# MinhZou/SNGNN

Measured on AMD Instinct MI355X. Metric: similarity-aggregation edges/sec, higher is better.
Workload: dtype f32; 1 GPU; ogbn-arxiv-sized synthetic graph, SNGNN_Plus aggregation forward, top_k=16, thr=0.0, self-loops removed; nodes_per_gpu=169343, edges_per_gpu=1163820, channels=40, parallelism=single GPU

## Files before the change

### include/sngnn_hip.h

```cpp
#ifndef SNGNN_HIP_H
#define SNGNN_HIP_H

#include <stdint.h>

#ifdef __cplusplus
extern "C" {
#endif

#define SNGNN_OK            0
#define SNGNN_EINVAL       -1
#define SNGNN_ERANGE       -2
#define SNGNN_EHIP         -3
#define SNGNN_ENOMEM       -4

#define SNGNN_UNSELECTED   (-4.0f)

#define SNGNN_MAX_CHANNELS  512

const char *sngnn_last_error(void);
const char *sngnn_build_info(void);

typedef struct sngnn_graph sngnn_graph_t;

#define SNGNN_LOOPS_REPLACE 2
int sngnn_graph_create(const int64_t *edge_index_dev, int64_t E, int64_t N,
                       int add_loops, int remove_loops, void *stream,
                       sngnn_graph_t **out_graph);
int sngnn_graph_create_partition(const int64_t *edge_index_dev, int64_t E,
                                 int64_t N_total, int64_t row_begin,
                                 int64_t row_end, int add_loops, int remove_loops,
                                 void *stream, sngnn_graph_t **out_graph);
void sngnn_graph_destroy(sngnn_graph_t *g);

int64_t sngnn_graph_num_nodes(const sngnn_graph_t *g);
int64_t sngnn_graph_num_total_nodes(const sngnn_graph_t *g);
int64_t sngnn_graph_row_offset(const sngnn_graph_t *g);
int64_t sngnn_graph_num_edges(const sngnn_graph_t *g);
int64_t sngnn_graph_max_in_degree(const sngnn_graph_t *g);
int64_t sngnn_graph_src_min(const sngnn_graph_t *g);
int64_t sngnn_graph_num_fused_nodes(const sngnn_graph_t *g);
int64_t sngnn_graph_workspace_bytes(const sngnn_graph_t *g, int C);

int sngnn_graph_copy_array(const sngnn_graph_t *g, int which, void *host_dst);
const void *sngnn_graph_array_dev(const sngnn_graph_t *g, int which);
int64_t sngnn_graph_array_len(const sngnn_graph_t *g, int which);

int sngnn_agg_forward(const sngnn_graph_t *g, const float *h, int C, int top_k,
                      float thr, float *out, float *wsel, float *inv_norm,
                      int32_t *sel_src, float *sel_w, void *workspace,
                      void *stream);

int sngnn_normalize_rows(const float *h, int64_t rows, int C, float *n, float *nrm,
                         void *stream);
int64_t sngnn_filter_row_bytes(int C);
int sngnn_normalize_rows_filter(const float *h, int64_t rows, int C, float *n, float *nrm,
                                void *filt, void *stream);
int sngnn_agg_forward_prepared(const sngnn_graph_t *g, const float *n, const float *nrm,
                               const void *filt, int C, int top_k, float thr, float *out,
                               float *wsel, float *inv_norm, int32_t *sel_src, float *sel_w,
                               void *workspace, void *stream);

typedef struct sngnn_epilogue {
    const float *bias;
    const unsigned char *keep;
    float keep_scale;
    int relu;
    const void *seed;
    float p;
    void *kept_bits;
    const int64_t *head_y;
    const unsigned char *head_sel;
    int head_sets;
    int head_out_mode;
    int64_t head_n_a, head_n_b;
    float *head_metrics;
    void *head_workspace;
    int no_filter;
} sngnn_epilogue_t;
int64_t sngnn_agg_head_workspace_bytes(const sngnn_graph_t *g);
int sngnn_agg_head_supported(const sngnn_graph_t *g, int C, int top_k);
int sngnn_agg_forward_epilogue(const sngnn_graph_t *g, const float *h, int C, int top_k, float thr,
                               const sngnn_epilogue_t *epi, float *out, float *wsel, float *inv_norm,
                               void *workspace, void *stream);
int sngnn_agg_forward_prepared_epilogue(const sngnn_graph_t *g, const float *n, const float *nrm,
                                        const void *filt, int C, int top_k, float thr,
                                        const sngnn_epilogue_t *epi, float *out, float *wsel,
                                        float *inv_norm, void *workspace, void *stream);
int sngnn_filter_enable(int mode);
int sngnn_filter_wanted(const sngnn_graph_t *g, int C, int top_k, float thr);
int sngnn_agg_forward_rows(const sngnn_graph_t *g, const float *n, const float *nrm,
                           const void *filt, int C, int top_k, float thr,
                           const uint8_t *row_flag, int row_want, float *out, float *wsel,
                           float *inv_norm, void *workspace, void *stream);
int sngnn_tuning_set(int which, int value);
int sngnn_last_forward_finalize_workgroups(void);
int sngnn_filter_pair_scores(const void *filt, int C, const int64_t *pair_a, const int64_t *pair_b,
                             int64_t n_pairs, float *out, void *stream);
int sngnn_agg_forward_normalized(const sngnn_graph_t *g, const float *n, const float *nrm,
                                 int C, int top_k, float thr, float *out, float *wsel,
                                 float *inv_norm, int32_t *sel_src, float *sel_w,
                                 void *workspace, void *stream);

int sngnn_agg_backward(const sngnn_graph_t *g, const float *h, int C,
                       const float *grad_out, const float *wsel, float *grad_h,
                       void *workspace, void *stream);
int sngnn_agg_backward_topk(const sngnn_graph_t *g, const float *h, int C,
                            const float *grad_out, const float *wsel, int top_k, float *grad_h,
                            void *workspace, void *stream);
int sngnn_agg_kept_bits_supported(const sngnn_graph_t *g, int C, int top_k);
int64_t sngnn_graph_kept_bits_bytes(const sngnn_graph_t *g);
int sngnn_agg_backward_bits(const sngnn_graph_t *g, const float *h, int C, const float *grad_out,
                            const void *kept_bits, int top_k, float *grad_h, void *workspace, void *stream);

#define SNGNN_DTYPE_F16 1
#define SNGNN_DTYPE_BF16 2
int sngnn_agg_forward_half(const sngnn_graph_t *g, const void *h, int dtype, int C, int top_k, float thr,
                           void *out, float *wsel, float *inv_norm, int32_t *sel_src, float *sel_w,
                           void *workspace, void *stream);
int sngnn_agg_backward_half(const sngnn_graph_t *g, const void *h, int dtype, int C, const void *grad_out,
                            const float *wsel, int top_k, void *grad_h, void *workspace, void *stream);

int sngnn_attn_forward(const sngnn_graph_t *g, const float *h, int C, float *out,
                       float *alpha, void *workspace, void *stream);
int sngnn_attn_backward(const sngnn_graph_t *g, const float *h, int C,
                        const float *grad_out, const float *alpha, float *grad_h,
                        void *workspace, void *stream);

int sngnn_signed_forward(const sngnn_graph_t *g, const float *wh, int C, const float *coef,
                         const float *c2, float *out, float *s, void *workspace, void *stream);
int sngnn_signed_backward(const sngnn_graph_t *g, const float *wh, int C, const float *grad_out,
                          const float *coef, const float *s, const float *c2, float *grad_wh, float *u,
                          void *workspace, void *stream);

int sngnn_attn_forward_half(const sngnn_graph_t *g, const void *h, int dtype, int C, void *out,
                            float *alpha, void *workspace, void *stream);
int sngnn_attn_backward_half(const sngnn_graph_t *g, const void *h, int dtype, int C, const void *grad_out,
                             const float *alpha, void *grad_h, void *workspace, void *stream);
int sngnn_signed_forward_half(const sngnn_graph_t *g, const void *wh, int dtype, int C, const float *coef,
                              const float *c2, void *out, float *s, void *workspace, void *stream);
int sngnn_signed_backward_half(const sngnn_graph_t *g, const void *wh, int dtype, int C, const void *grad_out,
                               const float *coef, const float *s, const float *c2, void *grad_wh, float *u,
                               void *workspace, void *stream);

int64_t sngnn_blend_workspace_bytes(void);
int sngnn_blend_forward(const float *out0, const float *out1, const float *beta, int64_t n,
                        float *out, void *stream);
int sngnn_blend_backward(const float *grad_out, const float *out0, const float *out1,
                         const float *beta, int64_t n, float *grad0, float *grad1,
                         float *grad_beta, void *workspace, void *stream);
int sngnn_blend_forward_epilogue(const float *out0, const float *out1, const float *beta, int64_t n,
                                 const sngnn_epilogue_t *epi, float *out, void *stream);
int sngnn_blend_backward_epilogue(const float *grad_out, const float *out0, const float *out1,
                                  const float *beta, int64_t n, const float *act, float scale,
                                  float *grad0, float *grad1, float *grad_beta, void *workspace,
                                  void *stream);

#define SNGNN_GGCN_ACT       1
#define SNGNN_GGCN_PREV_ELU  2
int64_t sngnn_ggcn_transition_workspace_bytes(void);
int sngnn_ggcn_transition_forward(const float *prop, const float *wh, const float *cs, const float *prev,
                                  float coeff, int flags, int64_t n, float *out, void *stream);
int sngnn_ggcn_transition_backward(const float *grad_out, const float *prop, const float *wh, const float *cs,
                                   const float *prev, float coeff, int flags, int64_t n, float *grad_prop,
                                   float *grad_wh, float *grad_prev, float *grad_cs, void *workspace, void *stream);

int64_t sngnn_bn_train_workspace_bytes(int C);
int sngnn_bn_train_forward(const float *x, const float *bias, int64_t N, int C, const float *gamma, const float *beta,
                           double eps, double momentum, float *running_mean, float *running_var,
                           const unsigned char *keep, float keep_scale, const void *seed, float p, float *out,
                           float *save_mean, float *save_invstd, void *workspace, void *stream);
int sngnn_bn_train_backward(const float *grad_out, const float *x, const float *bias, int64_t N, int C,
                            const float *gamma, const float *save_mean, const float *save_invstd,
                            const unsigned char *keep, float keep_scale, const void *seed, float p, float *grad_x,
                            float *grad_gamma, float *grad_beta, float *grad_bias, void *workspace, void *stream);
int sngnn_bn_post_forward(const float *x, int64_t N, int C, const float *gamma, const float *beta, double eps,
                          double momentum, float *running_mean, float *running_var, const unsigned char *keep,
                          float keep_scale, const void *seed, float p, float *out, float *save_mean,
                          float *save_invstd, void *workspace, void *stream);
int sngnn_bn_post_backward(const float *grad_out, const float *x, int64_t N, int C, const float *gamma,
                           const float *beta, const float *save_mean, const float *save_invstd,
                           const unsigned char *keep, float keep_scale, const void *seed, float p, float *grad_x,
                           float *grad_gamma, float *grad_beta, void *workspace, void *stream);

int sngnn_gather_sum_rows(const sngnn_graph_t *g, const float *table, const float *bias,
                          int C, float *out, void *workspace, void *stream);
int sngnn_scatter_sum_rows(const sngnn_graph_t *g, const float *vals, int C, float *out,
                           void *workspace, void *stream);
int sngnn_weighted_gather_sum_rows(const sngnn_graph_t *g, const float *table, const float *w_csr, int C,
                                   float *out, void *workspace, void *stream);
int sngnn_weighted_scatter_sum_rows(const sngnn_graph_t *g, const float *vals, const float *w_csc, int C,
                                    float *out, void *workspace, void *stream);
int sngnn_pair_dot_rows(const float *a_rows, const int32_t *idx_a, const float *b_rows, const int32_t *idx_b,
                        int64_t n_pairs, int C, float *out, void *stream);

int sngnn_prop_dinv(const sngnn_graph_t *g, float *dinv, void *stream);
int64_t sngnn_prop_workspace_bytes(const sngnn_graph_t *g, int C, int K);
int sngnn_prop_gpr_forward(const sngnn_graph_t *g, const float *x, const float *gamma, int K, int C,
                           const float *dinv, float *out, void *workspace, void *stream);
int sngnn_prop_gpr_backward(const sngnn_graph_t *g, const float *grad_out, const float *x, const float *gamma,
                            int K, int C, const float *dinv, float *grad_x, double *grad_gamma,
                            void *workspace, void *stream);
int sngnn_prop_appnp(const sngnn_graph_t *g, const float *h, const float *coef, int K, int C, const float *dinv,
                     int transpose, float *out, void *workspace, void *stream);

int64_t sngnn_gat_workspace_bytes(const sngnn_graph_t *g, int H, int C);
int sngnn_gat_scores(const float *xp, const float *att_src, const float *att_dst, int64_t N, int H, int C,
                     float *a_src, float *a_dst, void *stream);
int sngnn_gat_forward(const sngnn_graph_t *g, const float *xp, const float *a_src, const float *a_dst, int H, int C,
                      float negative_slope, float *out, float *ml, void *workspace, void *stream);
int sngnn_gat_backward(const sngnn_graph_t *g, const float *grad_out, const float *xp, const float *out,
                       const float *a_src, const float *a_dst, const float *ml, const float *att_src,
                       const float *att_dst, int H, int C, float negative_slope, float *grad_xp, float *grad_att,
                       void *workspace, void *stream);

int64_t sngnn_wrgat_workspace_bytes(const sngnn_graph_t *g, int R, int C);
int sngnn_wrgat_forward(const sngnn_graph_t *g, const float *P, int64_t P_stride, const float *self_rows,
                        int64_t self_stride, const float *bias, const int32_t *rel_ptr, const float *w_csr,
                        const float *atten, int R, int C, float negative_slope, int relu, float *out, float *scores,
                        float *ml, void *workspace, void *stream);
int sngnn_wrgat_backward(const sngnn_graph_t *g, const float *grad_out, const float *out, const float *P,
                         int64_t P_stride, const int32_t *rel_ptr, const int32_t *rel_csc, const float *w_csr,
                         const float *atten, const float *scores, const float *ml, int R, int C,
                         float negative_slope, int relu, float *grad_P, int64_t grad_P_stride, float *grad_self,
                         int64_t grad_self_stride, float *grad_atten, float *grad_bias, void *workspace, void *stream);

int64_t sngnn_acm_workspace_bytes(const sngnn_graph_t *g, int C);
int sngnn_acm_forward(const sngnn_graph_t *g, const float *P, const float *a_low, const float *a_high,
                      const float *a_mlp, const float *att_vec, int C, int relu, float *out, float *LH, float *datt,
                      void *workspace, void *stream);
int sngnn_acm_backward(const sngnn_graph_t *g, const float *grad_out, const float *P, const float *LH,
                       const float *datt, const float *a_low, const float *a_high, const float *a_mlp,
                       const float *att_vec, int C, int relu, float *grad_P, double *grad_params, void *workspace,
                       void *stream);

#define SNGNN_GCN2_MAX_C 128
int64_t sngnn_gcn2_workspace_bytes(const sngnn_graph_t *g, int C);
int sngnn_gcn2_hop(const sngnn_graph_t *g, const float *x, const float *x0, const float *dinv, float a, float b,
                   int C, int transpose, float *out, void *workspace, void *stream);
int sngnn_gcn2_map(const float *s, const float *w, float c0, float c1, int64_t N, int C, int transpose_w,
                   const float *rm, const float *invstd, const float *gamma, const float *beta_bn, float *out,
                   void *stream);

typedef struct sngnn_gcn_hop {
    const float *src;       int64_t ld_src;
    int W, W0;
    float *dst0;            int64_t ld0;
    float *dst1;            int64_t ld1;
    const float *pass_src;  int64_t ld_ps;
    float *pass_dst;        int64_t ld_pd;
    int Wp;
    int relu;
    const float *bias, *rm, *invstd, *gamma, *beta_bn;
} sngnn_gcn_hop_t;
int64_t sngnn_gcn_workspace_bytes(const sngnn_graph_t *g, int W);
int sngnn_gcn_hop(const sngnn_graph_t *g, const sngnn_gcn_hop_t *a, const float *dinv, int transpose,
                  void *workspace, void *stream);
int sngnn_gcn_bias_grad(const float *g, int64_t N, int C, float *grad_bias, void *workspace, void *stream);

#define SNGNN_TWO_HOP_HASH_MAX 1024
typedef struct sngnn_h2gcn_hop {
    const float *src;  int64_t ld_src;
    float *dst;        int64_t ld_dst;
    int W;
    const float *rm, *invstd, *gamma, *beta_bn;
} sngnn_h2gcn_hop_t;
int64_t sngnn_two_hop_workspace_bytes(const sngnn_graph_t *g);
int sngnn_two_hop_count(const sngnn_graph_t *g, int32_t *count, void *workspace, void *stream);
int sngnn_two_hop_fill(const sngnn_graph_t *g, const int64_t *offsets, int64_t E2, int64_t *edge_index,
                       void *workspace, void *stream);
int sngnn_h2gcn_dinv(const sngnn_graph_t *g, float *dinv, void *stream);
int64_t sngnn_h2gcn_workspace_bytes(const sngnn_graph_t *g, int W);
int sngnn_h2gcn_hop(const sngnn_graph_t *g1, const sngnn_graph_t *g2, const sngnn_h2gcn_hop_t *a, const float *dinv1,
                    const float *dinv2, int transpose, void *workspace1, void *workspace2, void *stream);

#define SNGNN_GLOGNN_MAX_C 64
int64_t sngnn_glognn_gram_workspace_bytes(int C);
int sngnn_glognn_gram(const float *a, const float *a_sub, double sub_scale, const float *a2, const float *b, int64_t N,
                      int C, double *out, double *out2, void *workspace, void *stream);
int sngnn_glognn_solve(const double *G, const float *diag, double alpha, double beta, double gamma, int C, double *M,
                       double *T, double *V, double *W, float *MT32, void *stream);
int sngnn_glognn_solve_backward(const double *gM, const double *gT, double scale_m, double scale_t, const double *G,
                                const double *V, const double *W, const float *diag, double alpha, double beta,
                                double gamma, int C, double *gG2, double *grad_diag, double *tmp, void *stream);
int64_t sngnn_glognn_workspace_bytes(const sngnn_graph_t *g, int C, int orders);
int sngnn_glognn_forward(const sngnn_graph_t *g, const float *x, const float *h0, const float *MT32,
                         const float *orders_weight, int orders, double beta, double gamma, int C, float *S, float *out,
                         void *workspace, void *stream);
int sngnn_glognn_backward(const sngnn_graph_t *g, const float *grad_out, const float *x, const float *MT32,
                          const double *gG2, const float *orders_weight, int orders, double beta, double gamma, int C,
                          float *grad_x, float *grad_h0, double *grad_w, void *workspace, void *stream);

#define SNGNN_LINKX_MAX_H 128
int sngnn_linkx_join_supported(int H);
int sngnn_linkx_join_forward(const float *zA, const float *zX, const float *W, const float *b, int64_t N, int H, int lsm,
                             float *ax, float *y, void *stream);
int sngnn_linkx_join_backward(const float *grad_y, const float *y, const float *ax, const float *W, int64_t N, int H,
                              int lsm, float *g, float *grad_zA, float *grad_zX, void *stream);

#define SNGNN_JK_MAX_LAYERS 8
int sngnn_jk_max_forward(const float *const *xs, int L, int64_t N, int C, float *out, unsigned char *which, void *stream);
int sngnn_jk_max_backward(const float *grad_out, const unsigned char *which, int L, int64_t N, int C, float *const *grads,
                          void *stream);

int sngnn_profile_enable(int on);
int sngnn_profile_last_forward(float *norm_ms, float *main_ms, float *fin_ms, float *empty_ms);
int64_t sngnn_gather_floor_workspace_bytes(void);
int sngnn_gather_floor(const sngnn_graph_t *g, const float *table, int C, int mode, float *out,
                       void *workspace, void *stream);

int sngnn_adj_linear_forward(const sngnn_graph_t *g, const float *wt,
                             const float *bias, int C, float *out0,
                             void *workspace, void *stream);
int sngnn_adj_linear_backward(const sngnn_graph_t *g, const float *g0, int C,
                              float *dwt, void *workspace, void *stream);

int64_t sngnn_head_workspace_bytes(int64_t N);
int sngnn_head_nll(const float *logits, const int64_t *y, const unsigned char *row_mask,
                   int64_t N, int C, int64_t n_masked, float *grad_logits,
                   float *loss_and_correct, void *workspace, void *stream);
int sngnn_head_nll2(const float *logits, const int64_t *y, const unsigned char *row_sets,
                    int64_t N, int C, int64_t n_a, int64_t n_b, float *out4, void *workspace,
                    void *stream);
int sngnn_head_nll_blend_supported(int C);
int sngnn_head_nll_blend(const float *out0, const float *out1, const float *beta, const int64_t *y,
                         const unsigned char *sel, int64_t N, int C, int sets, int64_t n_a, int64_t n_b,
                         float *grad_logits, float *logits_out, float *metrics, void *workspace, void *stream);
int sngnn_linear_forward(const float *x, const float *weight, const float *bias,
                         int64_t N, int F, int C, float *h, void *stream);
int sngnn_linear_forward_masked(const float *x, const float *weight, const float *bias, int64_t N,
                                int F, int C, const float *act, float act_scale, float *h, void *stream);
int sngnn_epilogue_backward(const float *grad, const float *act, float scale, int64_t n, float *grad_pre,
                            void *stream);
int sngnn_linear_normalized_supported(int64_t N, int F, int C);
int sngnn_linear_forward_normalized(const float *x, const float *weight, const float *bias,
                                    int64_t N, int F, int C, float *h, float *n, float *nrm,
                                    void *filt, void *stream);
int64_t sngnn_linear_wgrad_workspace_bytes(int64_t N, int C, int F);
int sngnn_linear_wgrad(const float *grad_out, const float *x, int64_t N, int C, int F,
                       float *grad_weight, float *grad_bias, void *workspace, void *stream);

int sngnn_cosine_dense(const float *x, int64_t N, int64_t F, float *S, void *stream);
int sngnn_cosine_class_sums(const float *x, int64_t N, int64_t F, const int32_t *y,
                            int n_classes, double *class_sum, double *diag_sum,
                            void *stream);
int64_t sngnn_cosine_hist_workspace_bytes(int64_t N, int64_t F, int bins, int groups);
int sngnn_cosine_hist(const float *x, int64_t N, int64_t F, const int32_t *y, const float *edges, int bins,
                      unsigned long long *counts, double *stats, void *workspace, void *stream);
int sngnn_edge_cosine(const float *x, int64_t N, int64_t F,
                      const int64_t *edge_index_dev, int64_t E, float *sim,
                      void *stream);
int sngnn_segment_mean(const float *val, const int64_t *index, int64_t E, int64_t M, float *mean,
                       int32_t *count, void *stream);
int sngnn_sparse_pair_dot(const int64_t *colptr, const int32_t *rowidx, const float *vals,
                          int64_t n_cols, const int64_t *pair_a, const int64_t *pair_b,
                          int64_t n_pairs, float *out, void *stream);

int64_t sngnn_knn_workspace_bytes(int64_t N, int k);
int sngnn_knn_graph(const float *x, int64_t N, int64_t F, int k, int exclude_self,
                    int32_t *nbr_idx, float *nbr_sim, void *workspace, void *stream);

int sngnn_replica_unpack(const float *hs, const float *bias, int64_t N, int R, int C, float *h, float *n,
                         float *nrm, void *filt, void *stream);
int64_t sngnn_replica_wgrad_workspace_bytes(int64_t N, int R, int C, int F);
int sngnn_replica_wgrad(const float *grad_out, const float *x, int64_t N, int R, int C, int F,
                        float *grad_weight, float *grad_bias, void *workspace, void *stream);
int64_t sngnn_replica_head_workspace_bytes(int R);
int sngnn_replica_head_nll(const float *logits, const float *logits1, const float *beta, const int64_t *y,
                           const unsigned char *sel, const int64_t *counts, int64_t N, int R, int C, int sets,
                           float *grad_logits, float *metrics, int64_t metrics_stride, void *workspace,
                           void *stream);
int64_t sngnn_replica_blend_workspace_bytes(int R);
int sngnn_replica_blend_forward(const float *out0, const float *out1, const float *beta, int64_t n, int R,
                                float *out, void *stream);
int sngnn_replica_blend_backward(const float *grad_out, const float *out0, const float *out1,
                                 const float *beta, int64_t n, int R, float *grad0, float *grad1,
                                 float *grad_beta, void *workspace, void *stream);

#ifdef __cplusplus
}
#endif
#endif
```

### sngnn_amd/_lib.py

```python
from __future__ import annotations

import ctypes as C
import os

import torch
from torch import Tensor

_HERE = os.path.dirname(os.path.abspath(__file__))
LIB_PATH = os.environ.get("SNGNN_LIB_PATH") or os.path.join(_HERE, "libsngnn_hip.so")

OK, EINVAL, ERANGE, EHIP, ENOMEM = 0, -1, -2, -3, -4
DTYPE_F16, DTYPE_BF16 = 1, 2
UNSELECTED = -4.0
LOOPS_REPLACE = 2
MAX_CHANNELS = 512
TWO_HOP_HASH_MAX = 1024

_vp, _i64, _i32, _f32, _f64 = C.c_void_p, C.c_int64, C.c_int, C.c_float, C.c_double

SIGNATURES = {
    "sngnn_last_error": (C.c_char_p, []), "sngnn_build_info": (C.c_char_p, []),
    "sngnn_graph_create": (_i32, [_vp, _i64, _i64, _i32, _i32, _vp, C.POINTER(_vp)]),
    "sngnn_graph_create_partition": (_i32, [_vp, _i64, _i64, _i64, _i64, _i32, _i32, _vp, C.POINTER(_vp)]),
    "sngnn_graph_destroy": (None, [_vp]),
    "sngnn_graph_num_nodes": (_i64, [_vp]), "sngnn_graph_num_total_nodes": (_i64, [_vp]),
    "sngnn_graph_row_offset": (_i64, [_vp]), "sngnn_graph_num_edges": (_i64, [_vp]),
    "sngnn_graph_max_in_degree": (_i64, [_vp]), "sngnn_graph_src_min": (_i64, [_vp]),
    "sngnn_graph_num_fused_nodes": (_i64, [_vp]), "sngnn_graph_workspace_bytes": (_i64, [_vp, _i32]),
    "sngnn_graph_copy_array": (_i32, [_vp, _i32, _vp]),
    "sngnn_graph_array_dev": (_vp, [_vp, _i32]), "sngnn_graph_array_len": (_i64, [_vp, _i32]),
    "sngnn_agg_forward": (_i32, [_vp, _vp, _i32, _i32, _f32, _vp, _vp, _vp, _vp, _vp, _vp, _vp]),
    "sngnn_normalize_rows": (_i32, [_vp, _i64, _i32, _vp, _vp, _vp]),
    "sngnn_filter_row_bytes": (_i64, [_i32]),
    "sngnn_normalize_rows_filter": (_i32, [_vp, _i64, _i32, _vp, _vp, _vp, _vp]),
    "sngnn_agg_forward_prepared": (_i32, [_vp, _vp, _vp, _vp, _i32, _i32, _f32, _vp, _vp, _vp, _vp, _vp, _vp, _vp]),
    "sngnn_agg_forward_epilogue": (_i32, [_vp, _vp, _i32, _i32, _f32, _vp, _vp, _vp, _vp, _vp, _vp]),
    "sngnn_agg_forward_prepared_epilogue": (_i32, [_vp, _vp, _vp, _vp, _i32, _i32, _f32, _vp, _vp, _vp, _vp, _vp, _vp]),
    "sngnn_filter_enable": (_i32, [_i32]),
    "sngnn_filter_wanted": (_i32, [_vp, _i32, _i32, _f32]),
    "sngnn_agg_forward_rows": (_i32, [_vp, _vp, _vp, _vp, _i32, _i32, _f32, _vp, _i32, _vp, _vp, _vp, _vp, _vp]),
    "sngnn_tuning_set": (_i32, [_i32, _i32]),
    "sngnn_last_forward_finalize_workgroups": (_i32, []),
    "sngnn_filter_pair_scores": (_i32, [_vp, _i32, _vp, _vp, _i64, _vp, _vp]),
    "sngnn_agg_forward_normalized": (_i32, [_vp, _vp, _vp, _i32, _i32, _f32, _vp, _vp, _vp, _vp, _vp, _vp, _vp]),
    "sngnn_agg_backward": (_i32, [_vp, _vp, _i32, _vp, _vp, _vp, _vp, _vp]),
    "sngnn_agg_backward_topk": (_i32, [_vp, _vp, _i32, _vp, _vp, _i32, _vp, _vp, _vp]),
    "sngnn_agg_kept_bits_supported": (_i32, [_vp, _i32, _i32]),
    "sngnn_agg_head_supported": (_i32, [_vp, _i32, _i32]),
    "sngnn_agg_head_workspace_bytes": (_i64, [_vp]),
    "sngnn_graph_kept_bits_bytes": (_i64, [_vp]),
    "sngnn_agg_backward_bits": (_i32, [_vp, _vp, _i32, _vp, _vp, _i32, _vp, _vp, _vp]),
    "sngnn_agg_forward_half": (_i32, [_vp, _vp, _i32, _i32, _i32, _f32, _vp, _vp, _vp, _vp, _vp, _vp, _vp]),
    "sngnn_agg_backward_half": (_i32, [_vp, _vp, _i32, _i32, _vp, _vp, _i32, _vp, _vp, _vp]),
    "sngnn_attn_forward": (_i32, [_vp, _vp, _i32, _vp, _vp, _vp, _vp]),
    "sngnn_attn_backward": (_i32, [_vp, _vp, _i32, _vp, _vp, _vp, _vp, _vp]),
    "sngnn_signed_forward": (_i32, [_vp, _vp, _i32, _vp, _vp, _vp, _vp, _vp, _vp]),
    "sngnn_signed_backward": (_i32, [_vp, _vp, _i32, _vp, _vp, _vp, _vp, _vp, _vp, _vp, _vp]),
    "sngnn_attn_forward_half": (_i32, [_vp, _vp, _i32, _i32, _vp, _vp, _vp, _vp]),
    "sngnn_attn_backward_half": (_i32, [_vp, _vp, _i32, _i32, _vp, _vp, _vp, _vp, _vp]),
    "sngnn_signed_forward_half": (_i32, [_vp, _vp, _i32, _i32, _vp, _vp, _vp, _vp, _vp, _vp]),
    "sngnn_signed_backward_half": (_i32, [_vp, _vp, _i32, _i32, _vp, _vp, _vp, _vp, _vp, _vp, _vp, _vp]),
    "sngnn_blend_workspace_bytes": (_i64, []), "sngnn_blend_forward": (_i32, [_vp, _vp, _vp, _i64, _vp, _vp]),
    "sngnn_blend_backward": (_i32, [_vp, _vp, _vp, _vp, _i64, _vp, _vp, _vp, _vp, _vp]),
    "sngnn_blend_forward_epilogue": (_i32, [_vp, _vp, _vp, _i64, _vp, _vp, _vp]),
    "sngnn_blend_backward_epilogue": (_i32, [_vp, _vp, _vp, _vp, _i64, _vp, _f32, _vp, _vp, _vp, _vp, _vp]),
    "sngnn_ggcn_transition_workspace_bytes": (_i64, []),
    "sngnn_ggcn_transition_forward": (_i32, [_vp, _vp, _vp, _vp, _f32, _i32, _i64, _vp, _vp]),
    "sngnn_ggcn_transition_backward": (_i32, [_vp, _vp, _vp, _vp, _vp, _f32, _i32, _i64, _vp, _vp, _vp, _vp, _vp, _vp]),
    "sngnn_bn_train_workspace_bytes": (_i64, [_i32]),
    "sngnn_bn_train_forward": (_i32, [_vp, _vp, _i64, _i32, _vp, _vp, C.c_double, C.c_double, _vp, _vp, _vp, _f32, _vp, _f32] + [_vp] * 5),
    "sngnn_bn_train_backward": (_i32, [_vp, _vp, _vp, _i64, _i32] + [_vp] * 4 + [_f32, _vp, _f32] + [_vp] * 6),
    "sngnn_bn_post_forward": (_i32, [_vp, _i64, _i32, _vp, _vp, C.c_double, C.c_double, _vp, _vp, _vp, _f32, _vp, _f32] + [_vp] * 5),
    "sngnn_bn_post_backward": (_i32, [_vp, _vp, _i64, _i32] + [_vp] * 5 + [_f32, _vp, _f32] + [_vp] * 5),
    "sngnn_knn_workspace_bytes": (_i64, [_i64, _i32]),
    "sngnn_knn_graph": (_i32, [_vp, _i64, _i64, _i32, _i32, _vp, _vp, _vp, _vp]),
    "sngnn_gather_sum_rows": (_i32, [_vp, _vp, _vp, _i32, _vp, _vp, _vp]),
    "sngnn_scatter_sum_rows": (_i32, [_vp, _vp, _i32, _vp, _vp, _vp]),
    "sngnn_weighted_gather_sum_rows": (_i32, [_vp, _vp, _vp, _i32, _vp, _vp, _vp]),
    "sngnn_weighted_scatter_sum_rows": (_i32, [_vp, _vp, _vp, _i32, _vp, _vp, _vp]),
    "sngnn_pair_dot_rows": (_i32, [_vp, _vp, _vp, _vp, _i64, _i32, _vp, _vp]),
    "sngnn_prop_dinv": (_i32, [_vp, _vp, _vp]), "sngnn_prop_workspace_bytes": (_i64, [_vp, _i32, _i32]),
    "sngnn_prop_gpr_forward": (_i32, [_vp, _vp, _vp, _i32, _i32, _vp, _vp, _vp, _vp]),
    "sngnn_prop_gpr_backward": (_i32, [_vp, _vp, _vp, _vp, _i32, _i32, _vp, _vp, _vp, _vp, _vp]),
    "sngnn_prop_appnp": (_i32, [_vp, _vp, _vp, _i32, _i32, _vp, _i32, _vp, _vp, _vp]),
    "sngnn_gat_workspace_bytes": (_i64, [_vp, _i32, _i32]), "sngnn_gat_scores": (_i32, [_vp, _vp, _vp, _i64, _i32, _i32, _vp, _vp, _vp]),
    "sngnn_gat_forward": (_i32, [_vp, _vp, _vp, _vp, _i32, _i32, _f32, _vp, _vp, _vp, _vp]),
    "sngnn_gat_backward": (_i32, [_vp] * 9 + [_i32, _i32, _f32, _vp, _vp, _vp, _vp]),
    "sngnn_wrgat_workspace_bytes": (_i64, [_vp, _i32, _i32]),
    "sngnn_wrgat_forward": (_i32, [_vp, _vp, _i64, _vp, _i64] + [_vp] * 4 + [_i32, _i32, _f32, _i32] + [_vp] * 5),
    "sngnn_wrgat_backward": (_i32, [_vp] * 4 + [_i64] + [_vp] * 6 + [_i32, _i32, _f32, _i32, _vp, _i64, _vp, _i64] + [_vp] * 4),
    "sngnn_acm_workspace_bytes": (_i64, [_vp, _i32]),
    "sngnn_acm_forward": (_i32, [_vp] * 6 + [_i32, _i32, _vp, _vp, _vp, _vp, _vp]),
    "sngnn_acm_backward": (_i32, [_vp] * 9 + [_i32, _i32, _vp, _vp, _vp, _vp]),
    "sngnn_gcn2_workspace_bytes": (_i64, [_vp, _i32]),
    "sngnn_gcn2_hop": (_i32, [_vp, _vp, _vp, _vp, _f32, _f32, _i32, _i32, _vp, _vp, _vp]),
    "sngnn_gcn2_map": (_i32, [_vp, _vp, _f32, _f32, _i64, _i32, _i32] + [_vp] * 6),
    "sngnn_gcn_workspace_bytes": (_i64, [_vp, _i32]), "sngnn_gcn_hop": (_i32, [_vp, _vp, _vp, _i32, _vp, _vp]),
    "sngnn_gcn_bias_grad": (_i32, [_vp, _i64, _i32, _vp, _vp, _vp]),
    "sngnn_two_hop_workspace_bytes": (_i64, [_vp]), "sngnn_two_hop_count": (_i32, [_vp, _vp, _vp, _vp]),
    "sngnn_two_hop_fill": (_i32, [_vp, _vp, _i64, _vp, _vp, _vp]),
    "sngnn_h2gcn_dinv": (_i32, [_vp, _vp, _vp]), "sngnn_h2gcn_workspace_bytes": (_i64, [_vp, _i32]),
    "sngnn_h2gcn_hop": (_i32, [_vp, _vp, _vp, _vp, _vp, _i32, _vp, _vp, _vp]),
    "sngnn_glognn_gram_workspace_bytes": (_i64, [_i32]), "sngnn_glognn_gram": (_i32, [_vp, _vp, _f64, _vp, _vp, _i64, _i32, _vp, _vp, _vp, _vp]),
    "sngnn_glognn_solve": (_i32, [_vp, _vp, _f64, _f64, _f64, _i32] + [_vp] * 6),
    "sngnn_glognn_solve_backward": (_i32, [_vp, _vp, _f64, _f64] + [_vp] * 4 + [_f64] * 3 + [_i32] + [_vp] * 4),
    "sngnn_glognn_workspace_bytes": (_i64, [_vp, _i32, _i32]), "sngnn_glognn_forward": (_i32, [_vp] * 5 + [_i32, _f64, _f64, _i32] + [_vp] * 4),
    "sngnn_glognn_backward": (_i32, [_vp] * 6 + [_i32, _f64, _f64, _i32] + [_vp] * 5),
    "sngnn_linkx_join_supported": (_i32, [_i32]), "sngnn_linkx_join_forward": (_i32, [_vp, _vp, _vp, _vp, _i64, _i32, _i32, _vp, _vp, _vp]),
    "sngnn_linkx_join_backward": (_i32, [_vp, _vp, _vp, _vp, _i64, _i32, _i32, _vp, _vp, _vp, _vp]),
    "sngnn_jk_max_forward": (_i32, [_vp, _i32, _i64, _i32, _vp, _vp, _vp]), "sngnn_jk_max_backward": (_i32, [_vp, _vp, _i32, _i64, _i32, _vp, _vp]),
    "sngnn_profile_enable": (_i32, [_i32]),
    "sngnn_profile_last_forward": (_i32, [C.POINTER(_f32), C.POINTER(_f32), C.POINTER(_f32), C.POINTER(_f32)]),
    "sngnn_gather_floor_workspace_bytes": (_i64, []), "sngnn_gather_floor": (_i32, [_vp, _vp, _i32, _i32, _vp, _vp, _vp]),
    "sngnn_adj_linear_forward": (_i32, [_vp, _vp, _vp, _i32, _vp, _vp, _vp]),
    "sngnn_adj_linear_backward": (_i32, [_vp, _vp, _i32, _vp, _vp, _vp]),
    "sngnn_head_workspace_bytes": (_i64, [_i64]),
    "sngnn_head_nll": (_i32, [_vp, _vp, _vp, _i64, _i32, _i64, _vp, _vp, _vp, _vp]),
    "sngnn_head_nll2": (_i32, [_vp, _vp, _vp, _i64, _i32, _i64, _i64, _vp, _vp, _vp]),
    "sngnn_head_nll_blend_supported": (_i32, [_i32]),
    "sngnn_head_nll_blend": (_i32, [_vp, _vp, _vp, _vp, _vp, _i64, _i32, _i32, _i64, _i64, _vp, _vp, _vp, _vp, _vp]),
    "sngnn_linear_forward": (_i32, [_vp, _vp, _vp, _i64, _i32, _i32, _vp, _vp]),
    "sngnn_linear_forward_masked": (_i32, [_vp, _vp, _vp, _i64, _i32, _i32, _vp, _f32, _vp, _vp]),
    "sngnn_epilogue_backward": (_i32, [_vp, _vp, _f32, _i64, _vp, _vp]),
    "sngnn_linear_normalized_supported": (_i32, [_i64, _i32, _i32]),
    "sngnn_linear_forward_normalized": (_i32, [_vp, _vp, _vp, _i64, _i32, _i32, _vp, _vp, _vp, _vp, _vp]),
    "sngnn_linear_wgrad_workspace_bytes": (_i64, [_i64, _i32, _i32]),
    "sngnn_linear_wgrad": (_i32, [_vp, _vp, _i64, _i32, _i32, _vp, _vp, _vp, _vp]),
    "sngnn_cosine_dense": (_i32, [_vp, _i64, _i64, _vp, _vp]),
    "sngnn_cosine_class_sums": (_i32, [_vp, _i64, _i64, _vp, _i32, _vp, _vp, _vp]),
    "sngnn_cosine_hist_workspace_bytes": (_i64, [_i64, _i64, _i32, _i32]),
    "sngnn_cosine_hist": (_i32, [_vp, _i64, _i64, _vp, _vp, _i32, _vp, _vp, _vp, _vp]),
    "sngnn_edge_cosine": (_i32, [_vp, _i64, _i64, _vp, _i64, _vp, _vp]),
    "sngnn_segment_mean": (_i32, [_vp, _vp, _i64, _i64, _vp, _vp, _vp]),
    "sngnn_sparse_pair_dot": (_i32, [_vp, _vp, _vp, _i64, _vp, _vp, _i64, _vp, _vp]),
    "sngnn_replica_unpack": (_i32, [_vp, _vp, _i64, _i32, _i32, _vp, _vp, _vp, _vp, _vp]),
    "sngnn_replica_wgrad_workspace_bytes": (_i64, [_i64, _i32, _i32, _i32]),
    "sngnn_replica_wgrad": (_i32, [_vp, _vp, _i64, _i32, _i32, _i32, _vp, _vp, _vp, _vp]),
    "sngnn_replica_head_workspace_bytes": (_i64, [_i32]),
    "sngnn_replica_head_nll": (_i32, [_vp, _vp, _vp, _vp, _vp, _vp, _i64, _i32, _i32, _i32, _vp, _vp, _i64, _vp, _vp]),
    "sngnn_replica_blend_workspace_bytes": (_i64, [_i32]),
    "sngnn_replica_blend_forward": (_i32, [_vp, _vp, _vp, _i64, _i32, _vp, _vp]),
    "sngnn_replica_blend_backward": (_i32, [_vp, _vp, _vp, _vp, _i64, _i32, _vp, _vp, _vp, _vp, _vp]),
}

STREAMLESS = ("sngnn_graph_copy_array",)


class Epilogue(C.Structure):
    _fields_ = [("bias", C.c_void_p), ("keep", C.c_void_p), ("keep_scale", C.c_float), ("relu", C.c_int),
                ("seed", C.c_void_p), ("p", C.c_float), ("kept_bits", C.c_void_p),
                ("head_y", C.c_void_p), ("head_sel", C.c_void_p), ("head_sets", C.c_int), ("head_out_mode", C.c_int),
                ("head_n_a", C.c_int64), ("head_n_b", C.c_int64), ("head_metrics", C.c_void_p),
                ("head_workspace", C.c_void_p), ("no_filter", C.c_int)]


class GcnHop(C.Structure):
    _fields_ = [("src", C.c_void_p), ("ld_src", C.c_int64), ("W", C.c_int), ("W0", C.c_int),
                ("dst0", C.c_void_p), ("ld0", C.c_int64), ("dst1", C.c_void_p), ("ld1", C.c_int64),
                ("pass_src", C.c_void_p), ("ld_ps", C.c_int64), ("pass_dst", C.c_void_p), ("ld_pd", C.c_int64),
                ("Wp", C.c_int), ("relu", C.c_int), ("bias", C.c_void_p), ("rm", C.c_void_p), ("invstd", C.c_void_p),
                ("gamma", C.c_void_p), ("beta_bn", C.c_void_p)]


class H2gcnHop(C.Structure):
    _fields_ = [("src", C.c_void_p), ("ld_src", C.c_int64), ("dst", C.c_void_p), ("ld_dst", C.c_int64), ("W", C.c_int),
                ("rm", C.c_void_p), ("invstd", C.c_void_p), ("gamma", C.c_void_p), ("beta_bn", C.c_void_p)]


_lib = None
_entries = {}


class SngnnError(RuntimeError):
    pass


def load():
    global _lib
    if _lib is None:
        if not os.path.exists(LIB_PATH):
            raise SngnnError(
                f"{LIB_PATH} is missing: build it with `python -c 'import __graft_entry__ as g; "
                f"g.build()'` or `make -C sngnn_amd/csrc` (there is no CPU fallback)")
        lib = C.CDLL(LIB_PATH)
        for name, (res, args) in SIGNATURES.items():
            fn = getattr(lib, name)
            fn.restype = res
            fn.argtypes = args
            if res is _i32 and args and args[-1] is _vp and name not in STREAMLESS:
                _entries[name] = fn
        _lib = lib
    return _lib


def check(rc: int, what: str) -> None:
    if rc != 0:
        msg = load().sngnn_last_error().decode("utf-8", "replace")
        exc = ValueError if rc in (EINVAL, ERANGE) else SngnnError
        raise exc(f"{what} failed ({rc}): {msg}")


def ptr(t):
    return None if t is None else t.data_ptr()


_guard, _current_stream = torch.cuda.device, torch.cuda.current_stream


def _ordinal(device):
    idx = getattr(device, "index", None)
    return device if idx is None else idx


def stream(device) -> int:
    return _current_stream(_ordinal(device)).cuda_stream


def _entry(name):
    load()
    if name not in _entries:
        raise SngnnError(f"{name} is not a status entry that takes the stream last")
    return _entries[name]


def call(name, device, *args):
    try:
        fn = _entries[name]
    except KeyError:
        fn = _entry(name)
    ptrs = []
    add = ptrs.append
    for a in args:
        if type(a) is Tensor or isinstance(a, Tensor):
            if not a.is_contiguous():
                raise ValueError(f"{name}: argument {len(ptrs) + 1} must be a contiguous tensor, got shape "
                                 f"{tuple(a.shape)} with strides {a.stride()}")
            a = a.data_ptr()
        add(a)
    idx = _ordinal(device)
    with _guard(idx):
        rc = fn(*ptrs, _current_stream(idx).cuda_stream)
    if rc != 0:
        check(rc, name)


_ws_cache = {}


def workspace(key, nbytes, device):
    held = _ws_cache.setdefault((key, str(device), stream(device) if torch.device(device).type == "cuda" else None), [])
    if not held or held[-1].numel() < nbytes:
        held.append(torch.empty(max(int(nbytes), 256, 2 * held[-1].numel() if held else 0), dtype=torch.uint8, device=device))
    return held[-1]
```

### sngnn_amd/csrc/agg_bwd.hip

```cpp
#include "agg_bwd_impl.h"
#include "entry.h"

using namespace sngnn;

static int g_bwd_mode = 0, g_bwd_roles = 3;
int sngnn::set_bwd_mode(int v) { g_bwd_mode = (v == 1 || v == 2) ? v : 0; return SNGNN_OK; }
int sngnn::set_bwd_roles(int v) { g_bwd_roles = v & 7; return SNGNN_OK; }

extern "C" int sngnn_agg_backward(const sngnn_graph_t *g, const float *h, int C,
                                  const float *grad_out, const float *wsel, float *grad_h,
                                  void *workspace, void *stream)
{
    return sngnn_agg_backward_topk(g, h, C, grad_out, wsel, -1, grad_h, workspace, stream);
}

static bool node_centric(const sngnn_graph_t *g)
{
    const bool mostly_fused = (int64_t)g->n_fused * 2 >= g->N;
    return g_bwd_mode == 2 || (g_bwd_mode == 0 && mostly_fused);
}
bool sngnn::kept_bits_path(const sngnn_graph_t *g, int top_k)
{
    return g != nullptr && g->csc_bit != nullptr && g->N == g->Ntot && top_k >= 1 && top_k <= SMALL_T && node_centric(g) &&
           !fwd_scores_on_the_fly_forced();
}

static int backward_impl(const sngnn_graph_t *g, const float *h, int C, const float *grad_out, const float *wsel,
                         const unsigned *kbits, int top_k, float *grad_h, void *workspace, void *stream,
                         int dtype = 0);

extern "C" int sngnn_agg_backward_topk(const sngnn_graph_t *g, const float *h, int C,
                                       const float *grad_out, const float *wsel, int top_k,
                                       float *grad_h, void *workspace, void *stream)
{
    SN_REQUIRE(g == nullptr || wsel != nullptr || g->Ep == 0, SNGNN_EINVAL, "wsel is NULL");
    return backward_impl(g, h, C, grad_out, wsel, nullptr, top_k, grad_h, workspace, stream);
}

extern "C" int sngnn_agg_backward_bits(const sngnn_graph_t *g, const float *h, int C, const float *grad_out,
                                       const void *kept_bits, int top_k, float *grad_h, void *workspace,
                                       void *stream)
{
    SN_REQUIRE(g != nullptr && kept_bits != nullptr, SNGNN_EINVAL, "graph / kept_bits is NULL");
    SN_REQUIRE(kept_bits_path(g, top_k), SNGNN_EINVAL,
               "no kept-bit path for this graph / top_k (sngnn_agg_kept_bits_supported)");
    return backward_impl(g, h, C, grad_out, nullptr, (const unsigned *)kept_bits, top_k, grad_h, workspace, stream);
}

extern "C" int sngnn_agg_backward_half(const sngnn_graph_t *g, const void *h, int dtype, int C, const void *grad_out,
                                       const float *wsel, int top_k, void *grad_h, void *workspace, void *stream)
{
    SN_REQUIRE(dtype == SNGNN_DTYPE_F16 || dtype == SNGNN_DTYPE_BF16, SNGNN_EINVAL,
               "dtype must be SNGNN_DTYPE_F16 or SNGNN_DTYPE_BF16");
    SN_REQUIRE(g == nullptr || wsel != nullptr || g->Ep == 0, SNGNN_EINVAL, "wsel is NULL");
    return backward_impl(g, (const float *)h, C, (const float *)grad_out, wsel, nullptr, top_k, (float *)grad_h,
                         workspace, stream, dtype);
}

static int backward_impl(const sngnn_graph_t *g, const float *h, int C, const float *grad_out, const float *wsel,
                         const unsigned *kbits, int top_k, float *grad_h, void *workspace, void *stream, int dtype)
{
    SN_REQUIRE(g != nullptr, SNGNN_EINVAL, "graph is NULL");
    if (g->Ntot == 0) return SNGNN_OK;
    SN_REQUIRE(h && grad_h && workspace && (grad_out || g->N == 0), SNGNN_EINVAL, "NULL argument");
    RowCfg cfg;
    if (int rc = check_rows(C, dtype, {h, grad_out, grad_h}, cfg)) return rc;
    const BwdLayout L = bwd_layout(g, C, false);
    BwdArgs a;
    bind_bwd_graph(g, C, L, workspace, a);
    a.h = h; a.gout = grad_out; a.wsel = wsel; a.grad_h = grad_h;
    a.wd = nullptr; a.rec_dot = nullptr;
    a.kmask = (unsigned *)((char *)workspace + L.rec);
    a.kmask_words = (g->Ep + 31) / 32;
    a.inv_deg = g->inv_deg;
    a.mode = node_centric(g) ? 0 : 1;
    a.top_k = top_k;
    a.role_mask = g_bwd_roles;
    a.fdesc = g->fdesc; a.trest = g->trest;
    a.n_fused = g->n_fused; a.n_trest = g->n_trest;
    a.kbits = kbits; a.csc_bit = g->csc_bit; a.kb_wbase = (int)g->kb_wbase; a.kb_tbase = (int)g->kb_tbase;
    a.s_small_end = a.mode == 0 ? g->srcs_gt(SMALL_T - 1) : (int)g->Ntot;
    return SNGNN_LAUNCH_VEC(launch_agg_bwd_vec, cfg, dtype, a, (hipStream_t)stream);
}
```

### sngnn_amd/csrc/agg_bwd_impl.h

```cpp
#pragma once
#include "device_utils.h"

#ifndef SNGNN_BWDF_STEP
#define SNGNN_BWDF_STEP 1
#endif

namespace sngnn {

struct BwdArgs {
    const float *h, *gout, *wsel;
    int C, N, Ntot, row_off;
    const int32_t *rowptr, *col, *rperm;
    const int4 *rdesc, *sdesc;
    const int32_t *cscptr, *csc_eid, *csc_dst, *csc_pos, *sperm;
    float2 *wd;
    float *rec_dot;
    unsigned *kmask;
    int64_t kmask_words, Ep;
    const float *inv_deg;
    float *dnT, *grad_h;
    int n_split, n_med_end, n_tasks;
    const int32_t *task_slot, *task_chunk, *split_task0;
    float *partT;
    int n_ssplit, n_smed_end, n_stasks;
    const int32_t *stask_slot, *stask_chunk, *ssplit_task0;
    float *partS;
    int nbA, nbB;
    int s_small_end;
    const int4 *fdesc;
    const int4 *trest;
    int n_fused, n_trest, nbC;
    int mode;
    int role_mask;
    int top_k;
    const unsigned *kbits;
    const int32_t *csc_bit;
    int kb_wbase, kb_tbase;
    template <typename S> __device__ __forceinline__ const S *hrows() const { return reinterpret_cast<const S *>(h); }
    template <typename S> __device__ __forceinline__ const S *grows() const { return reinterpret_cast<const S *>(gout); }
    template <typename S> __device__ __forceinline__ S *dhrows() const { return reinterpret_cast<S *>(grad_h); }
};

__device__ __forceinline__ bool kbit(const BwdArgs &a, int b) { return (a.kbits[b >> 5] >> (b & 31)) & 1u; }

__device__ __forceinline__ bool is_kept(float w) { return w > -3.0f; }

template <int G> __device__ __forceinline__ unsigned long long group_bits(unsigned long long m, int gid)
{
    if constexpr (G == 64) return m;
    else return (m >> (gid * G)) & ((1ull << G) - 1ull);
}

template <int VEC, int G, int R>
__device__ __forceinline__ void fma_row(Row<VEC, G, R> &acc, float w, const Row<VEC, G, R> &x)
{
#pragma unroll
    for (int r = 0; r < R; ++r)
#pragma unroll
        for (int v = 0; v < VEC; ++v) acc.x[r][v] = fmaf(w, x.x[r][v], acc.x[r][v]);
}

template <int VEC, int G, int R>
__device__ __forceinline__ void t_edge_row(const Row<VEC, G, R> &x, const Row<VEC, G, R> &gp,
                                           Row<VEC, G, R> &acc, float live = 1.0f)
{
    const float invj = inv_norm_of(group_sum<G>(x.dot_partial(x)));
    const float d = group_sum<G>(gp.dot_partial(x));
    fma_row<VEC, G, R>(acc, d * invj * live, x);
}

__device__ __forceinline__ bool kept_csr(const BwdArgs &a, int e) { return (a.kmask[e >> 5] >> (e & 31)) & 1u; }

template <bool KB> __device__ __forceinline__ bool kept_out(const BwdArgs &a, int q)
{
    if constexpr (KB) return kbit(a, a.csc_bit[q]);
    else return kept_csr(a, a.csc_eid[q]);
}

__device__ __forceinline__ void set_kept_bit(const BwdArgs &a, int cp)
{
    atomicOr(a.kmask + (cp >> 5), 1u << (cp & 31));
}

template <bool MARK>
__device__ __forceinline__ int kept_list(const BwdArgs &a, int rs, int e0, int e1, int *jlist)
{
    const int lane = lane_id();
    int n = 0;
    for (int base = e0; base < e1; base += 64) {
        const int t = base + lane;
        bool kept;
        int cp = 0;
        if constexpr (MARK) {
            const float w = t < e1 ? a.wsel[rs + t] : SNGNN_UNSELECTED;
            cp = t < e1 ? a.csc_pos[rs + t] : 0;
            kept = is_kept(w);
        } else {
            kept = t < e1 && kept_csr(a, rs + t);
        }
        const int j = t < e1 ? a.col[rs + t] : 0;
        const unsigned long long m = __ballot(kept);
        if (kept) {
            jlist[n + prefix_popc(m)] = j;
            if constexpr (MARK) set_kept_bit(a, cp);
        }
        n += __popcll(m);
    }
    return n;
}

template <int VEC, int G, int R, bool MARK, typename S = float>
__device__ __forceinline__ void t_role_small(const BwdArgs &a, int blk, int *lds_wave, const int4 *desc, int n_desc)
{
    using RowT = Row<VEC, G, R>;
    constexpr int RPW = 64 / G;
    const int lane = lane_id(), wave = threadIdx.x >> 6;
    const int gid = lane / G, lg = lane % G;
    const int slot = (blk * WAVES + wave) * RPW + gid;
    if (slot >= n_desc) return;
    const int4 d = desc[slot];
    const int i = d.x, rs = d.y, deg = d.z;
    int *s_j = lds_wave + gid * SMALL_T;
    const float invdeg = 1.0f / (float)max(deg, 1);
    int nk = 0;
    for (int t0 = 0; t0 < deg; t0 += G) {
        const int t = t0 + lg;
        bool kept;
        int cp = 0;
        if constexpr (MARK) {
            const float w = t < deg ? a.wsel[rs + t] : SNGNN_UNSELECTED;
            cp = t < deg ? a.csc_pos[rs + t] : 0;
            kept = is_kept(w);
        } else {
            kept = t < deg && kept_csr(a, rs + t);
        }
        const int j = t < deg ? a.col[rs + t] : 0;
        const unsigned long long gm = group_bits<G>(__ballot(kept), gid);
        if (kept) {
            s_j[nk + __popcll(gm & ((1ull << lg) - 1ull))] = j;
            if constexpr (MARK) set_kept_bit(a, cp);
        }
        nk += __popcll(gm);
    }
    RowT gp, acc;
    gp.load(a.grows<S>() + (size_t)i * a.C, a.C, lg);
    gp.scale(invdeg);
    acc.zero();
    wave_lds_sync();
    for (int q0 = 0; q0 < nk; q0 += 2) {
        const bool two = q0 + 1 < nk;
        const int q1 = two ? q0 + 1 : q0;
        RowT x0, x1;
        x0.load(a.hrows<S>() + (size_t)s_j[q0] * a.C, a.C, lg);
        x1.load(a.hrows<S>() + (size_t)s_j[q1] * a.C, a.C, lg);
        t_edge_row<VEC, G, R>(x0, gp, acc);
        t_edge_row<VEC, G, R>(x1, gp, acc, two ? 1.0f : 0.0f);
    }
    acc.store(a.dnT + (size_t)i * a.C, a.C, lg);
}

template <int VEC, int G, int R, bool MARK, typename S = float>
__device__ __forceinline__ void t_role_wave(const BwdArgs &a, int blk, int *lds_wave, bool task)
{
    using RowT = Row<VEC, G, R>;
    constexpr int NG = 64 / G;
    const int lane = lane_id(), wave = threadIdx.x >> 6;
    const int gid = lane / G, lg = lane % G;
    int i, e0, e1, tq = 0;
    int4 d;
    if (task) {
        tq = blk * WAVES + wave;
        if (tq >= a.n_tasks) return;
        d = a.rdesc[a.task_slot[tq]];
        e0 = a.task_chunk[tq] * CHUNK;
    } else {
        const int slot = a.n_split + blk * WAVES + wave;
        if (slot >= a.n_med_end) return;
        d = a.rdesc[slot];
        e0 = 0;
    }
    i = d.x;
    const int rs = d.y, deg = d.z;
    e1 = task ? min(deg, e0 + CHUNK) : deg;
    RowT gp, acc;
    const float invdeg = 1.0f / (float)deg;
    gp.load(a.grows<S>() + (size_t)i * a.C, a.C, lg);
    gp.scale(invdeg);
    acc.zero();
    int *jlist = lds_wave;
    const int nsel = kept_list<MARK>(a, rs, e0, e1, jlist);
    wave_lds_sync();
    for (int q0 = 0; q0 < nsel; q0 += 2 * NG) {
        const int qa = min(q0 + gid, nsel - 1), qb = min(q0 + NG + gid, nsel - 1);
        RowT xa, xb;
        xa.load(a.hrows<S>() + (size_t)jlist[qa] * a.C, a.C, lg);
        xb.load(a.hrows<S>() + (size_t)jlist[qb] * a.C, a.C, lg);
        t_edge_row<VEC, G, R>(xa, gp, acc, q0 + gid < nsel ? 1.0f : 0.0f);
        t_edge_row<VEC, G, R>(xb, gp, acc, q0 + NG + gid < nsel ? 1.0f : 0.0f);
    }
    acc.reduce_across_groups();
    if (gid == 0) {
        float *dst = task ? a.partT + (size_t)tq * a.C : a.dnT + (size_t)i * a.C;
        acc.store(dst, a.C, lg);
    }
}

template <int VEC, int G, int R, typename S = float>
__global__ __launch_bounds__(BLOCK) void k_bwd_t(const BwdArgs a)
{
    __shared__ __align__(16) int lds[WAVES][WAVE_T];
    const int b = blockIdx.x;
    int *lw = lds[threadIdx.x >> 6];
    if (b < a.nbA) t_role_wave<VEC, G, R, true, S>(a, b, lw, true);
    else if (b < a.nbA + a.nbB) t_role_wave<VEC, G, R, true, S>(a, b - a.nbA, lw, false);
    else t_role_small<VEC, G, R, true, S>(a, b - a.nbA - a.nbB, lw, a.rdesc + a.n_med_end, a.N - a.n_med_end);
}

static __global__ __launch_bounds__(256) void k_bwd_t_fin(const BwdArgs a)
{
    __shared__ float s[4][64];
    const int p = blockIdx.x;
    const int i = a.rperm[p];
    const int t0 = a.split_task0[p], t1 = a.split_task0[p + 1];
    const int cl = threadIdx.x & 63, q = threadIdx.x >> 6;
    for (int c0 = 0; c0 < a.C; c0 += 64) {
        const int c = c0 + cl;
        float v0 = 0.f, v1 = 0.f, v2 = 0.f, v3 = 0.f;
        if (c < a.C) {
            int t = t0 + q;
            for (; t + 12 < t1; t += 16) {
                v0 += a.partT[(size_t)t * a.C + c];
                v1 += a.partT[(size_t)(t + 4) * a.C + c];
                v2 += a.partT[(size_t)(t + 8) * a.C + c];
                v3 += a.partT[(size_t)(t + 12) * a.C + c];
            }
            for (; t < t1; t += 4) v0 += a.partT[(size_t)t * a.C + c];
        }
        s[q][cl] = (v0 + v1) + (v2 + v3);
        __syncthreads();
        if (q == 0 && c < a.C) a.dnT[(size_t)i * a.C + c] = (s[0][cl] + s[1][cl]) + (s[2][cl] + s[3][cl]);
        __syncthreads();
    }
}

template <int VEC, int G, int R>
__device__ __forceinline__ void s_edge(const BwdArgs &a, int i, float2 rec, int lg,
                                       Row<VEC, G, R> &msg, Row<VEC, G, R> &dns)
{
    Row<VEC, G, R> x, gi;
    x.load(a.h + (size_t)(i + a.row_off) * a.C, a.C, lg);
    gi.load(a.gout + (size_t)i * a.C, a.C, lg);
    const float invi = inv_norm_of(group_sum<G>(x.dot_partial(x)));
    fma_row<VEC, G, R>(msg, rec.x, gi);
    fma_row<VEC, G, R>(dns, rec.y * invi, x);
}

template <int VEC, int G, int R, typename S = float> struct FinishRows {
    Row<VEC, G, R> t, hv;
    bool own;
    __device__ __forceinline__ void load(const BwdArgs &a, int v, int lg)
    {
        const int vl = v - a.row_off;
        own = vl >= 0 && vl < a.N;
        t.load(a.dnT + (size_t)(own ? vl : 0) * a.C, a.C, lg);
        hv.load(a.hrows<S>() + (size_t)v * a.C, a.C, lg);
    }
};

template <int VEC, int G, int R, typename S = float>
__device__ __forceinline__ void s_finish(const BwdArgs &a, int v, int lg, Row<VEC, G, R> &msg,
                                         Row<VEC, G, R> &dn, FinishRows<VEC, G, R, S> &f)
{
    if (f.own) dn.add(f.t);
    Row<VEC, G, R> &hv = f.hv;
    const float qv = group_sum<G>(hv.dot_partial(hv));
    const float invv = inv_norm_of(qv);
    hv.scale(invv);
    float proj = group_sum<G>(hv.dot_partial(dn));
    if (norm_clamped(qv)) proj = 0.f;
#pragma unroll
    for (int r = 0; r < R; ++r)
#pragma unroll
        for (int c = 0; c < VEC; ++c)
            msg.x[r][c] += (dn.x[r][c] - hv.x[r][c] * proj) * invv;
    msg.store(a.dhrows<S>() + (size_t)v * a.C, a.C, lg);
}

template <int VEC, int G, int R>
__device__ __forceinline__ void s_edge_recompute(const Row<VEC, G, R> &x, const Row<VEC, G, R> &gi,
                                                 const Row<VEC, G, R> &hv, float invv, float invdeg,
                                                 float live, Row<VEC, G, R> &msg, Row<VEC, G, R> &dns)
{
    const float invi = inv_norm_of(group_sum<G>(x.dot_partial(x)));
    const float w = group_sum<G>(x.dot_partial(hv)) * (invi * invv);
    const float dse = group_sum<G>(gi.dot_partial(hv)) * invdeg;
    fma_row<VEC, G, R>(msg, w * invdeg * live, gi);
    fma_row<VEC, G, R>(dns, dse * invi * live, x);
}

template <int VEC, int G, int R>
__device__ __forceinline__ void s_edge_rows(const Row<VEC, G, R> &x, const Row<VEC, G, R> &gi,
                                            float w, float dse, Row<VEC, G, R> &msg,
                                            Row<VEC, G, R> &dns)
{
    const float invi = inv_norm_of(group_sum<G>(x.dot_partial(x)));
    fma_row<VEC, G, R>(msg, w, gi);
    fma_row<VEC, G, R>(dns, dse * invi, x);
}

template <int VEC, int G, int R, bool REC, bool CSRM, typename S = float>
__device__ __forceinline__ void s_role_small(const BwdArgs &a, int blk, int *lds_wave)
{
    using RowT = Row<VEC, G, R>;
    constexpr int RPW = 64 / G;
    const int lane = lane_id(), wave = threadIdx.x >> 6;
    const int gid = lane / G, lg = lane % G;
    const int slot = a.n_smed_end + (blk * WAVES + wave) * RPW + gid;
    if (slot >= a.s_small_end) return;
    const int4 d = a.sdesc[slot];
    const int v = d.x, qs = d.y, od = d.z;
    FinishRows<VEC, G, R, S> fin;
    fin.load(a, v, lg);
    int *s_i = lds_wave + gid * 3 * SMALL_T;
    float *s_w = reinterpret_cast<float *>(s_i + SMALL_T);
    float *s_ds = reinterpret_cast<float *>(s_i + 2 * SMALL_T);
    int nk = 0;
    for (int t0 = 0; t0 < od; t0 += G) {
        const int t = t0 + lg;
        float2 rec = make_float2(SNGNN_UNSELECTED, 0.f);
        int it = 0;
        bool kept = false;
        if (t < od) {
            const int q = qs + t;
            it = a.csc_dst[q];
            if constexpr (REC) rec = a.wd[q];
            else if constexpr (CSRM) kept = a.kbits ? kbit(a, a.csc_bit[q]) : kept_csr(a, a.csc_eid[q]);
            else kept = (a.kmask[q >> 5] >> (q & 31)) & 1u;
        }
        if constexpr (REC) kept = t < od;
        const unsigned long long gm = group_bits<G>(__ballot(kept), gid);
        if (kept) {
            const int pos = nk + __popcll(gm & ((1ull << lg) - 1ull));
            s_i[pos] = it;
            if constexpr (REC) { s_w[pos] = rec.x; s_ds[pos] = rec.y; }
        }
        nk += __popcll(gm);
    }
    RowT msg, dns;
    msg.zero();
    dns.zero();
    float invv = 0.f;
    if constexpr (!REC) invv = inv_norm_of(group_sum<G>(fin.hv.dot_partial(fin.hv)));
    wave_lds_sync();
    for (int q0 = 0; q0 < nk; q0 += 2) {
        const bool two = q0 + 1 < nk;
        const int q1 = two ? q0 + 1 : q0;
        const int i0 = s_i[q0], i1 = s_i[q1];
        RowT x0, g0, x1, g1;
        x0.load(a.hrows<S>() + (size_t)(i0 + a.row_off) * a.C, a.C, lg);
        g0.load(a.grows<S>() + (size_t)i0 * a.C, a.C, lg);
        x1.load(a.hrows<S>() + (size_t)(i1 + a.row_off) * a.C, a.C, lg);
        g1.load(a.grows<S>() + (size_t)i1 * a.C, a.C, lg);
        if constexpr (REC) {
            float w0 = s_w[q0], w1 = s_w[q1], ds0 = s_ds[q0], ds1 = s_ds[q1];
            if (a.rec_dot) {
                const bool r0 = (__float_as_uint(w0) >> 31) != 0, r1 = (__float_as_uint(w1) >> 31) != 0;
                const float t0_ = a.rec_dot[r0 ? i0 : 0], t1_ = a.rec_dot[r1 ? i1 : 0];
                w0 = fabsf(w0); w1 = fabsf(w1);
                ds0 = r0 ? w0 * (ds0 - t0_) : ds0;
                ds1 = r1 ? w1 * (ds1 - t1_) : ds1;
            }
            s_edge_rows<VEC, G, R>(x0, g0, w0, ds0, msg, dns);
            s_edge_rows<VEC, G, R>(x1, g1, two ? w1 : 0.f, two ? ds1 : 0.f, msg, dns);
        } else {
            const float d0 = a.inv_deg[(a.role_mask & 4) ? 0 : i0], d1 = a.inv_deg[(a.role_mask & 4) ? 0 : i1];
            s_edge_recompute<VEC, G, R>(x0, g0, fin.hv, invv, d0, 1.0f, msg, dns);
            s_edge_recompute<VEC, G, R>(x1, g1, fin.hv, invv, d1, two ? 1.0f : 0.0f, msg, dns);
        }
    }
    s_finish<VEC, G, R, S>(a, v, lg, msg, dns, fin);
}

template <int VEC, int G, int R, bool KB = false, typename S = float>
__device__ __forceinline__ void f_role_node(const BwdArgs &a, int blk, int *lds_wave)
{
    using RowT = Row<VEC, G, R>;
    constexpr int RPW = 64 / G;
    const int lane = lane_id(), wave = threadIdx.x >> 6;
    const int gid = lane / G, lg = lane % G;
    const int slot = (blk * WAVES + wave) * RPW + gid;
    if (slot >= a.n_fused) return;
    const int4 d = a.fdesc[slot];
    const int v = d.x, rs = d.y, qs = d.z, deg = d.w & 255, od = d.w >> 8;
    const int vl = v - a.row_off;
    int *s_j = lds_wave + gid * 2 * SMALL_T;
    int *s_i = s_j + SMALL_T;
    FinishRows<VEC, G, R, S> fin;
    RowT gp;
    gp.load(a.grows<S>() + (size_t)vl * a.C, a.C, lg);
    fin.hv.load(a.hrows<S>() + (size_t)v * a.C, a.C, lg);
    fin.own = true;
    int nk = 0, nko = 0;
    unsigned hw = 0u;
    if constexpr (KB) hw = reinterpret_cast<const unsigned short *>(a.kbits)[vl];
    for (int t0 = 0; t0 < max(deg, od); t0 += G) {
        const int t = t0 + lg;
        bool kept_i;
        if constexpr (KB) kept_i = t < deg && ((hw >> t) & 1u);
        else kept_i = t < deg && kept_csr(a, rs + t);
        const int j = t < deg ? a.col[rs + t] : 0;
        bool kept_o = false;
        int it = 0;
        if (t < od) {
            it = a.csc_dst[qs + t];
            kept_o = kept_out<KB>(a, qs + t);
        }
        const unsigned long long gi = group_bits<G>(__ballot(kept_i), gid);
        const unsigned long long go = group_bits<G>(__ballot(kept_o), gid);
        const unsigned long long below = (1ull << lg) - 1ull;
        if (kept_i) s_j[nk + __popcll(gi & below)] = j;
        if (kept_o) s_i[nko + __popcll(go & below)] = it;
        nk += __popcll(gi);
        nko += __popcll(go);
    }
    gp.scale(1.0f / (float)max(deg, 1));
    const float invv = inv_norm_of(group_sum<G>(fin.hv.dot_partial(fin.hv)));
    RowT msg, dns;
    fin.t.zero();
    msg.zero();
    dns.zero();
    wave_lds_sync();
    constexpr int FU = SNGNN_BWDF_STEP;
    const int steps = (max(nk, nko) + FU - 1) / FU;
    for (int s = 0; s < steps; ++s) {
        RowT xj[FU], x[FU], gi[FU];
        float dd[FU];
        bool ti[FU], to[FU];
#pragma unroll
        for (int u = 0; u < FU; ++u) {
            const int q = FU * s + u;
            ti[u] = q < nk;
            to[u] = q < nko;
            const int j = ti[u] ? s_j[q] : v;
            const int i = to[u] ? s_i[q] : vl;
            xj[u].load(a.hrows<S>() + (size_t)j * a.C, a.C, lg);
            x[u].load(a.hrows<S>() + (size_t)(i + a.row_off) * a.C, a.C, lg);
            gi[u].load(a.grows<S>() + (size_t)i * a.C, a.C, lg);
            dd[u] = a.inv_deg[i];
        }
#pragma unroll
        for (int u = 0; u < FU; ++u) t_edge_row<VEC, G, R>(xj[u], gp, fin.t, ti[u] ? 1.0f : 0.0f);
#pragma unroll
        for (int u = 0; u < FU; ++u)
            s_edge_recompute<VEC, G, R>(x[u], gi[u], fin.hv, invv, dd[u], to[u] ? 1.0f : 0.0f, msg, dns);
    }
    s_finish<VEC, G, R, S>(a, v, lg, msg, dns, fin);
}

__device__ __forceinline__ int wave_prefix_incl(int v)
{
    const int lane = lane_id();
#pragma unroll
    for (int d = 1; d < 64; d <<= 1) {
        const int o = __shfl_up(v, d, 64);
        if (lane >= d) v += o;
    }
    return v;
}

template <int VEC, int G, int R, bool KB = false, typename S = float>
__device__ __forceinline__ void w_role_node(const BwdArgs &a, int blk, int *lds_wave)
{
    using RowT = Row<VEC, G, R>;
    constexpr int NG = 64 / G;
    const int lane = lane_id(), wave = threadIdx.x >> 6;
    const int gid = lane / G, lg = lane % G;
    const int slot = blk * WAVES + wave;
    if (slot >= a.n_med_end + a.n_trest) return;
    const int4 d = slot < a.n_med_end ? a.rdesc[slot] : a.trest[slot - a.n_med_end];
    const int vl = d.x, rs = d.y, deg = d.z;
    const int v = vl + a.row_off;
    const int qs = a.cscptr[v], od = a.cscptr[v + 1] - qs;
    FinishRows<VEC, G, R, S> fin;
    RowT gp;
    gp.load(a.grows<S>() + (size_t)vl * a.C, a.C, lg);
    fin.hv.load(a.hrows<S>() + (size_t)v * a.C, a.C, lg);
    fin.own = true;
    gp.scale(1.0f / (float)max(deg, 1));
    fin.t.zero();
    int *elist = lds_wave;
    int *s_i = lds_wave + WAVE_T;
    int n = 0;
    bool have_ids = false;
    auto flush = [&]() {
        wave_lds_sync();
        if (!have_ids) {
            for (int t = lane; t < n; t += 64) elist[t] = a.col[(KB ? rs : 0) + elist[t]];
            wave_lds_sync();
        }
        for (int q0 = 0; q0 < n; q0 += 2 * NG) {
            const int qa = min(q0 + gid, n - 1), qb = min(q0 + NG + gid, n - 1);
            RowT xa, xb;
            xa.load(a.hrows<S>() + (size_t)elist[qa] * a.C, a.C, lg);
            xb.load(a.hrows<S>() + (size_t)elist[qb] * a.C, a.C, lg);
            t_edge_row<VEC, G, R>(xa, gp, fin.t, q0 + gid < n ? 1.0f : 0.0f);
            t_edge_row<VEC, G, R>(xb, gp, fin.t, q0 + NG + gid < n ? 1.0f : 0.0f);
        }
        wave_lds_sync();
        n = 0;
    };
    auto append = [&](unsigned word, int wi, int total) {
        if (n + total > WAVE_T) flush();
        const int cnt = __popc(word);
        int o = n + wave_prefix_incl(cnt) - cnt;
        while (word) {
            const int b = __builtin_ctz(word);
            word &= word - 1u;
            elist[o++] = wi * 32 + b;
        }
        n += total;
    };
    const int e_end = rs + deg;
    if (deg <= WAVE_T) {
        const int bitbase = !KB ? 0 : (slot < a.n_med_end ? 32 * (a.kb_wbase + 4 * (slot - a.n_split)) : 16 * vl);
        for (int base = 0; base < deg; base += 64) {
            const int t = base + lane;
            bool kept;
            if constexpr (KB) kept = t < deg && kbit(a, bitbase + t);
            else kept = t < deg && kept_csr(a, rs + t);
            const int j = t < deg ? a.col[rs + t] : 0;
            const unsigned long long m = __ballot(kept);
            if (kept) elist[n + prefix_popc(m)] = j;
            n += __popcll(m);
        }
        have_ids = true;
    } else if constexpr (KB) {
        const unsigned *rowbits = a.kbits + a.kb_tbase + 4 * a.split_task0[slot];
        const int nwords = 4 * (a.split_task0[slot + 1] - a.split_task0[slot]);
        for (int w0 = 0; w0 < nwords; w0 += 64) {
            const int wi = w0 + lane;
            const unsigned word = wi < nwords ? rowbits[wi] : 0u;
            const int total = wave_sum_i(__popc(word));
            if (total <= WAVE_T) append(word, wi, total);
            else
                for (int sb = 0; sb < 16; ++sb) {
                    const unsigned ws = (lane >> 2) == sb ? word : 0u;
                    append(ws, wi, wave_sum_i(__popc(ws)));
                }
        }
    } else {
        for (int w0 = rs >> 5; w0 * 32 < e_end; w0 += 64) {
            const int wi = w0 + lane;
            unsigned word = (int64_t)wi * 32 < e_end ? a.kmask[wi] : 0u;
            if (wi * 32 < rs) word &= ~0u << (rs & 31);
            if (wi * 32 + 32 > e_end) word &= wi * 32 >= e_end ? 0u : ~0u >> ((32 - (e_end & 31)) & 31);
            const int total = wave_sum_i(__popc(word));
            if (total <= WAVE_T) append(word, wi, total);
            else
                for (int sb = 0; sb < 16; ++sb) {
                    const unsigned ws = (lane >> 2) == sb ? word : 0u;
                    append(ws, wi, wave_sum_i(__popc(ws)));
                }
        }
    }
    int nso = 0;
    const bool s_here = od <= WAVE_T;
    if (s_here)
        for (int base = 0; base < od; base += 64) {
            const int t = base + lane;
            const int it = t < od ? a.csc_dst[qs + t] : 0;
            const bool kept = t < od && kept_out<KB>(a, qs + t);
            const unsigned long long m = __ballot(kept);
            if (kept) s_i[nso + prefix_popc(m)] = it;
            nso += __popcll(m);
        }
    if (n > 0) flush();
    fin.t.reduce_across_groups();
    if (!s_here) {
        if (gid == 0) fin.t.store(a.dnT + (size_t)vl * a.C, a.C, lg);
        return;
    }
    const float invv = inv_norm_of(group_sum<G>(fin.hv.dot_partial(fin.hv)));
    RowT msg, dns;
    msg.zero();
    dns.zero();
    wave_lds_sync();
    for (int q0 = 0; q0 < nso; q0 += 2 * NG) {
        const int qa = min(q0 + gid, nso - 1), qb = min(q0 + NG + gid, nso - 1);
        const bool la = q0 + gid < nso, lb = q0 + NG + gid < nso;
        const int ia = s_i[qa], ib = s_i[qb];
        RowT xa, ga, xb, gb;
        xa.load(a.hrows<S>() + (size_t)(ia + a.row_off) * a.C, a.C, lg);
        ga.load(a.grows<S>() + (size_t)ia * a.C, a.C, lg);
        xb.load(a.hrows<S>() + (size_t)(ib + a.row_off) * a.C, a.C, lg);
        gb.load(a.grows<S>() + (size_t)ib * a.C, a.C, lg);
        const float da = a.inv_deg[ia], db = a.inv_deg[ib];
        s_edge_recompute<VEC, G, R>(xa, ga, fin.hv, invv, da, la ? 1.0f : 0.0f, msg, dns);
        s_edge_recompute<VEC, G, R>(xb, gb, fin.hv, invv, db, lb ? 1.0f : 0.0f, msg, dns);
    }
    msg.reduce_across_groups();
    dns.reduce_across_groups();
    if (gid == 0) s_finish<VEC, G, R, S>(a, v, lg, msg, dns, fin);
}

static __global__ __launch_bounds__(256) void k_pack_kept(const float *__restrict__ wsel, int64_t Ep,
                                                          unsigned long long *__restrict__ kmask64)
{
    const int lane = lane_id();
    const int64_t base = (blockIdx.x * (int64_t)WAVES + (threadIdx.x >> 6)) * 256;
    if (base >= Ep) return;
    float w[4];
#pragma unroll
    for (int u = 0; u < 4; ++u) {
        const int64_t e = base + u * 64 + lane;
        w[u] = e < Ep ? wsel[e] : SNGNN_UNSELECTED;
    }
    unsigned long long m[4];
#pragma unroll
    for (int u = 0; u < 4; ++u) m[u] = __ballot(is_kept(w[u]));
    if (lane < 4 && base + lane * 64 < Ep) kmask64[(base >> 6) + lane] = lane == 0 ? m[0] : lane == 1 ? m[1] : lane == 2 ? m[2] : m[3];
}

#define SNGNN_BWDF_ATTR __attribute__((amdgpu_waves_per_eu(R == 1 ? 8 : 1, 8)))
template <int VEC, int G, int R, bool KB = false, typename S = float>
__global__ __launch_bounds__(BLOCK) SNGNN_BWDF_ATTR void k_bwd_w(const BwdArgs a)
{
    __shared__ __align__(16) int lds[WAVES][2 * WAVE_T];
    const int b = blockIdx.x;
    int *lw = lds[threadIdx.x >> 6];
    const int stride = a.nbB;
    const int cw = min(a.nbA, (b + stride - 1) / stride);
    if (b % stride == 0 && b / stride < a.nbA) { if (a.role_mask & 1) w_role_node<VEC, G, R, KB, S>(a, b / stride, lw); }
    else if (a.role_mask & 2) f_role_node<VEC, G, R, KB, S>(a, b - cw, lw);
}

template <int VEC, int G, int R, typename S = float>
__global__ __launch_bounds__(BLOCK) SNGNN_BWDF_ATTR void k_bwd_f(const BwdArgs a)
{
    __shared__ __align__(16) int lds[WAVES][256];
    const int b = blockIdx.x;
    int *lw = lds[threadIdx.x >> 6];
    if (b < a.nbA) t_role_wave<VEC, G, R, false, S>(a, b, lw, true);
    else if (b < a.nbA + a.nbB) t_role_wave<VEC, G, R, false, S>(a, b - a.nbA, lw, false);
    else if (b < a.nbA + a.nbB + a.nbC) t_role_small<VEC, G, R, false, S>(a, b - a.nbA - a.nbB, lw, a.trest, a.n_trest);
    else f_role_node<VEC, G, R, false, S>(a, b - a.nbA - a.nbB - a.nbC, lw);
}

template <int VEC, int G, int R, bool REC, bool CSRM, typename S = float>
__device__ __forceinline__ void s_role_wave(const BwdArgs &a, int blk, int *lds_wave, bool task)
{
    using RowT = Row<VEC, G, R>;
    constexpr int NG = 64 / G;
    const int lane = lane_id(), wave = threadIdx.x >> 6;
    const int gid = lane / G, lg = lane % G;
    int v, e0, tq = 0;
    int4 d;
    if (task) {
        tq = blk * WAVES + wave;
        if (tq >= a.n_stasks) return;
        d = a.sdesc[a.stask_slot[tq]];
        e0 = a.stask_chunk[tq] * CHUNK;
    } else {
        const int slot = a.n_ssplit + blk * WAVES + wave;
        if (slot >= a.n_smed_end) return;
        d = a.sdesc[slot];
        e0 = 0;
    }
    v = d.x;
    const int qs = d.y, od = d.z;
    const int e1 = task ? min(od, e0 + CHUNK) : od;
    RowT hv;
    float invv = 0.f;
    if constexpr (!REC) hv.load(a.hrows<S>() + (size_t)v * a.C, a.C, lg);
    int *s_i = lds_wave;
    float2 *s_rec = reinterpret_cast<float2 *>(lds_wave + WAVE_T);
    int nsel = 0;
    for (int base = e0; base < e1; base += 64) {
        const int t = base + lane;
        const int q = qs + t;
        float2 rec = make_float2(SNGNN_UNSELECTED, 0.f);
        const int it = t < e1 ? a.csc_dst[q] : 0;
        bool kept;
        if constexpr (REC) {
            if (t < e1) rec = a.wd[q];
            kept = t < e1;
        } else if constexpr (CSRM) {
            kept = t < e1 && (a.kbits ? kbit(a, a.csc_bit[q]) : kept_csr(a, a.csc_eid[q]));
        } else {
            kept = t < e1 && ((a.kmask[q >> 5] >> (q & 31)) & 1u);
        }
        const unsigned long long m = __ballot(kept);
        if (kept) {
            const int o = nsel + prefix_popc(m);
            s_i[o] = it;
            if constexpr (REC) s_rec[o] = rec;
        }
        nsel += __popcll(m);
    }
    if constexpr (!REC) invv = inv_norm_of(group_sum<G>(hv.dot_partial(hv)));
    wave_lds_sync();
    RowT msg, dns;
    msg.zero();
    dns.zero();
    for (int q0 = 0; q0 < nsel; q0 += 2 * NG) {
        const int qa = min(q0 + gid, nsel - 1), qb = min(q0 + NG + gid, nsel - 1);
        const bool la = q0 + gid < nsel, lb = q0 + NG + gid < nsel;
        const int ia = s_i[qa], ib = s_i[qb];
        RowT xa, ga, xb, gb;
        xa.load(a.hrows<S>() + (size_t)(ia + a.row_off) * a.C, a.C, lg);
        ga.load(a.grows<S>() + (size_t)ia * a.C, a.C, lg);
        xb.load(a.hrows<S>() + (size_t)(ib + a.row_off) * a.C, a.C, lg);
        gb.load(a.grows<S>() + (size_t)ib * a.C, a.C, lg);
        if constexpr (REC) {
            float2 ra = s_rec[qa], rb = s_rec[qb];
            if (a.rec_dot) {
                const bool wa = (__float_as_uint(ra.x) >> 31) != 0, wb = (__float_as_uint(rb.x) >> 31) != 0;
                const float da_ = a.rec_dot[wa ? ia : 0], db_ = a.rec_dot[wb ? ib : 0];
                ra.x = fabsf(ra.x); rb.x = fabsf(rb.x);
                ra.y = wa ? ra.x * (ra.y - da_) : ra.y;
                rb.y = wb ? rb.x * (rb.y - db_) : rb.y;
            }
            if (!la) ra = make_float2(0.f, 0.f);
            if (!lb) rb = make_float2(0.f, 0.f);
            s_edge_rows<VEC, G, R>(xa, ga, ra.x, ra.y, msg, dns);
            s_edge_rows<VEC, G, R>(xb, gb, rb.x, rb.y, msg, dns);
        } else {
            const float da = a.inv_deg[(a.role_mask & 4) ? 0 : ia], db = a.inv_deg[(a.role_mask & 4) ? 0 : ib];
            s_edge_recompute<VEC, G, R>(xa, ga, hv, invv, da, la ? 1.0f : 0.0f, msg, dns);
            s_edge_recompute<VEC, G, R>(xb, gb, hv, invv, db, lb ? 1.0f : 0.0f, msg, dns);
        }
    }
    msg.reduce_across_groups();
    dns.reduce_across_groups();
    if (task) {
        if (gid == 0) {
            msg.store(a.partS + (size_t)tq * 2 * a.C, a.C, lg);
            dns.store(a.partS + (size_t)tq * 2 * a.C + a.C, a.C, lg);
        }
    } else if (gid == 0) {
        FinishRows<VEC, G, R, S> fin;
        fin.load(a, v, lg);
        s_finish<VEC, G, R, S>(a, v, lg, msg, dns, fin);
    }
}

template <int VEC, int G, int R, bool REC, bool CSRM = false, typename S = float>
__global__ __launch_bounds__(BLOCK) void k_bwd_s(const BwdArgs a)
{
    __shared__ __align__(16) int lds[WAVES][512];
    const int b = blockIdx.x;
    int *lw = lds[threadIdx.x >> 6];
    if (b < a.nbA) s_role_wave<VEC, G, R, REC, CSRM, S>(a, b, lw, true);
    else if (b < a.nbA + a.nbB) s_role_wave<VEC, G, R, REC, CSRM, S>(a, b - a.nbA, lw, false);
    else s_role_small<VEC, G, R, REC, CSRM, S>(a, b - a.nbA - a.nbB, lw);
}

template <int VEC, int G, int R, typename S = float>
__global__ __launch_bounds__(64) void k_bwd_s_fin(const BwdArgs a)
{
    using RowT = Row<VEC, G, R>;
    const int lane = lane_id();
    const int gid = lane / G, lg = lane % G;
    const int p = blockIdx.x;
    const int v = a.sperm[p];
    const int t0 = a.ssplit_task0[p], t1 = a.ssplit_task0[p + 1];
    if (gid != 0) return;
    RowT msg, dns, t;
    msg.zero();
    dns.zero();
    for (int tq = t0; tq < t1; ++tq) {
        t.load(a.partS + (size_t)tq * 2 * a.C, a.C, lg);
        msg.add(t);
        t.load(a.partS + (size_t)tq * 2 * a.C + a.C, a.C, lg);
        dns.add(t);
    }
    FinishRows<VEC, G, R, S> fin;
    fin.load(a, v, lg);
    s_finish<VEC, G, R, S>(a, v, lg, msg, dns, fin);
}

static __global__ void k_clear_words(unsigned *__restrict__ p, int64_t n)
{
    for (int64_t i = blockIdx.x * (int64_t)blockDim.x + threadIdx.x; i < n; i += (int64_t)gridDim.x * blockDim.x) p[i] = 0u;
}

template <int VEC, int G, int R, typename S = float> int launch_agg_bwd(const BwdArgs &a0, hipStream_t st)
{
    constexpr int RPW = 64 / G;
    BwdArgs a = a0;
    if (a.mode == 0) {
        if (a.kmask_words > 0 && a.kbits == nullptr)
            k_pack_kept<<<ceil_div(a.Ep, 256 * WAVES), 256, 0, st>>>(a.wsel, a.Ep, (unsigned long long *)a.kmask);
        if (a.kbits != nullptr && !(a.top_k >= 1 && a.top_k <= WAVE_T && a.N == a.Ntot)) {
            set_error("internal: the kept-bit backward is the hinted node-centric one");
            return SNGNN_EINVAL;
        }
        if (a.top_k >= 1 && a.top_k <= WAVE_T && a.N == a.Ntot) {
            a.nbA = ceil_div(a.n_med_end + a.n_trest, WAVES);
            const int nbF = ceil_div(a.n_fused, (int64_t)WAVES * RPW);
            a.nbB = std::max(1, (a.nbA + nbF) / std::max(a.nbA, 1));
            if (a.nbA + nbF > 0) {
                if (a.kbits) k_bwd_w<VEC, G, R, true, S><<<a.nbA + nbF, BLOCK, 0, st>>>(a);
                else k_bwd_w<VEC, G, R, false, S><<<a.nbA + nbF, BLOCK, 0, st>>>(a);
            }
            if (a.n_stasks > 0) {
                a.nbA = ceil_div(a.n_stasks, WAVES);
                a.nbB = 0;
                k_bwd_s<VEC, G, R, false, true, S><<<a.nbA, BLOCK, 0, st>>>(a);
                k_bwd_s_fin<VEC, G, R, S><<<a.n_ssplit, 64, 0, st>>>(a);
            }
            SN_HIP(hipGetLastError());
            return SNGNN_OK;
        }
        a.nbA = ceil_div(a.n_tasks, WAVES);
        a.nbB = ceil_div(a.n_med_end - a.n_split, WAVES);
        a.nbC = ceil_div(a.n_trest, (int64_t)WAVES * RPW);
        const int nbD = ceil_div(a.n_fused, (int64_t)WAVES * RPW);
        if (a.nbA + a.nbB + a.nbC + nbD > 0) k_bwd_f<VEC, G, R, S><<<a.nbA + a.nbB + a.nbC + nbD, BLOCK, 0, st>>>(a);
        if (a.n_split > 0) k_bwd_t_fin<<<a.n_split, 256, 0, st>>>(a);
        a.nbA = ceil_div(a.n_stasks, WAVES);
        a.nbB = ceil_div(a.n_smed_end - a.n_ssplit, WAVES);
        const int nbS = ceil_div(a.s_small_end - a.n_smed_end, (int64_t)WAVES * RPW);
        if (a.nbA + a.nbB + nbS > 0) k_bwd_s<VEC, G, R, false, true, S><<<a.nbA + a.nbB + nbS, BLOCK, 0, st>>>(a);
        if (a.n_ssplit > 0) k_bwd_s_fin<VEC, G, R, S><<<a.n_ssplit, 64, 0, st>>>(a);
        SN_HIP(hipGetLastError());
        return SNGNN_OK;
    }
    if (a.kmask_words > 0)
        k_clear_words<<<(int)std::min<int64_t>(ceil_div(a.kmask_words, (int64_t)256), 1024), 256, 0, st>>>(a.kmask, a.kmask_words);
    a.nbA = ceil_div(a.n_tasks, WAVES);
    a.nbB = ceil_div(a.n_med_end - a.n_split, WAVES);
    int nbC = ceil_div(a.N - a.n_med_end, (int64_t)WAVES * RPW);
    if (a.nbA + a.nbB + nbC > 0) k_bwd_t<VEC, G, R, S><<<a.nbA + a.nbB + nbC, BLOCK, 0, st>>>(a);
    if (a.n_split > 0) k_bwd_t_fin<<<a.n_split, 256, 0, st>>>(a);
    a.nbA = ceil_div(a.n_stasks, WAVES);
    a.nbB = ceil_div(a.n_smed_end - a.n_ssplit, WAVES);
    nbC = ceil_div(a.s_small_end - a.n_smed_end, (int64_t)WAVES * RPW);
    if (a.nbA + a.nbB + nbC > 0) k_bwd_s<VEC, G, R, false, false, S><<<a.nbA + a.nbB + nbC, BLOCK, 0, st>>>(a);
    if (a.n_ssplit > 0) k_bwd_s_fin<VEC, G, R, S><<<a.n_ssplit, 64, 0, st>>>(a);
    SN_HIP(hipGetLastError());
    return SNGNN_OK;
}

template <typename S, int VEC> int launch_agg_bwd_vec(const RowCfg &cfg, const BwdArgs &a, hipStream_t st);

}

#define SNGNN_AGG_BWD_TU(S, VEC)                                                                                       \
    template <> int sngnn::launch_agg_bwd_vec<S, VEC>(const RowCfg &cfg, const BwdArgs &a, hipStream_t st)             \
    {                                                                                                                  \
        SNGNN_DISPATCH_GRS(launch_agg_bwd, VEC, S, cfg, a, st)                                                         \
    }
```

### sngnn_amd/csrc/agg_bwd_v1.hip

```cpp
#include "agg_bwd_impl.h"

SNGNN_AGG_BWD_TU(float, 1)
```

### sngnn_amd/csrc/agg_bwd_v2.hip

```cpp
#include "agg_bwd_impl.h"

SNGNN_AGG_BWD_TU(float, 2)
```

### sngnn_amd/csrc/agg_bwd_v4.hip

```cpp
#include "agg_bwd_impl.h"

SNGNN_AGG_BWD_TU(float, 4)
```

### sngnn_amd/csrc/agg_fwd.hip

```cpp
#include <atomic>
#include "agg_fwd_args.h"
#include "agg_fwd_filter.h"
#include "fwd_plan.h"
#include "head_row.h"
#include "entry.h"

using namespace sngnn;

static bool g_prof_on = false;
namespace sngnn { int g_prof_reps = 1; }
static hipEvent_t g_prof_ev[5] = {nullptr, nullptr, nullptr, nullptr, nullptr};

extern "C" int sngnn_profile_enable(int on)
{
    if (on && !g_prof_ev[0])
        for (auto &e : g_prof_ev) SN_HIP(hipEventCreate(&e));
    g_prof_on = on != 0;
    g_prof_reps = on > 1 ? on : 1;
    return SNGNN_OK;
}

extern "C" int sngnn_profile_last_forward(float *norm_ms, float *main_ms, float *fin_ms, float *empty_ms)
{
    SN_REQUIRE(g_prof_ev[0] != nullptr && norm_ms && main_ms && fin_ms && empty_ms, SNGNN_EINVAL,
               "profiling is not enabled");
    SN_HIP(hipEventSynchronize(g_prof_ev[4]));
    SN_HIP(hipEventElapsedTime(norm_ms, g_prof_ev[0], g_prof_ev[1]));
    SN_HIP(hipEventElapsedTime(main_ms, g_prof_ev[1], g_prof_ev[2]));
    SN_HIP(hipEventElapsedTime(fin_ms, g_prof_ev[2], g_prof_ev[3]));
    SN_HIP(hipEventElapsedTime(empty_ms, g_prof_ev[3], g_prof_ev[4]));
    *norm_ms /= (float)g_prof_reps;
    *main_ms /= (float)g_prof_reps;
    *fin_ms /= (float)g_prof_reps;
    return SNGNN_OK;
}

static __global__ void k_fill_sel(int32_t *__restrict__ src, float *__restrict__ w, int64_t n)
{
    for (int64_t i = blockIdx.x * (int64_t)blockDim.x + threadIdx.x; i < n; i += (int64_t)gridDim.x * blockDim.x) {
        src[i] = -1;
        w[i] = 0.f;
    }
}

static int normalize_dispatch(const RowCfg &cfg, const float *h, int64_t rows, int C, float *n, float *nrm,
                              void *filt, hipStream_t st)
{
    return dispatch_vec(cfg, [&](auto vec) {
        return launch_normalize_vec<float, decltype(vec)::value>(cfg, h, rows, C, n, nrm, filt, st);
    });
}

constexpr int FILT_MIN_DEG = 32;
constexpr double FILT_PRUNABLE_SHARE = 0.62;
static int g_filter_mode = 1;
static int g_role_mask = 7;
static int g_table_mode = 0;
static int g_filt_min_deg = -1;
int sngnn::g_fin_inline = 1;
static int g_addr_mode = 0;
int sngnn::g_last_fin_blocks = 0;
extern "C" int sngnn_last_forward_finalize_workgroups(void) { return sngnn::g_last_fin_blocks; }
unsigned long long sngnn::next_fin_nonce()
{
    static std::atomic<unsigned long long> counter{0};
    return 0xF1A0000000000000ull + counter.fetch_add(1) + 1;
}
bool sngnn::fwd_scores_on_the_fly_forced() { return g_table_mode == 2; }
extern "C" int sngnn_tuning_set(int which, int value)
{
    SN_REQUIRE(which == 0 || (which >= 2 && which <= 11), SNGNN_EINVAL, "unknown tuning knob");
    if (which == 11) { g_addr_mode = value == 1 ? 1 : 0; return SNGNN_OK; }
    if (which == 10) return sngnn::set_hist_copies(value);
    if (which == 9) { sngnn::g_fin_inline = value < 0 ? 0 : value; return SNGNN_OK; }
    if (which == 8) { g_filt_min_deg = value; return SNGNN_OK; }
    if (which == 7) return sngnn::set_cosine_split(value);
    if (which == 6) return sngnn::set_knn_route(value);
    if (which == 5) return sngnn::set_lin_mode(value);
    if (which == 3) return sngnn::set_bwd_mode(value);
    if (which == 4) return sngnn::set_bwd_roles(value);
    if (which == 0) g_role_mask = value & 7;
    else g_table_mode = value;
    return SNGNN_OK;
}

extern "C" int sngnn_filter_enable(int mode)
{
    SN_REQUIRE(mode >= 0 && mode <= 3, SNGNN_EINVAL,
               "filter mode must be 0 (off), 1 (auto), 2 (always) or 3 (wave rows and tasks always)");
    g_filter_mode = mode;
    return SNGNN_OK;
}

extern "C" int64_t sngnn_filter_row_bytes(int C) { return filter_row_bytes(C); }

extern "C" int sngnn_normalize_rows_filter(const float *h, int64_t rows, int C, float *n, float *nrm, void *filt,
                                           void *stream)
{
    SN_REQUIRE(rows >= 0, SNGNN_EINVAL, "negative row count");
    SN_REQUIRE(rows == 0 || (h && n && nrm), SNGNN_EINVAL, "h/n/nrm is NULL");
    RowCfg cfg;
    if (int rc = check_rows(C, 0, {h, n}, cfg)) return rc;
    SN_REQUIRE(filt == nullptr || filter_row_bytes(C) > 0, SNGNN_EINVAL,
               "no filter rows for this C (sngnn_filter_row_bytes(C) == 0)");
    SN_REQUIRE(((uintptr_t)filt % 16) == 0, SNGNN_EINVAL, "filt must be 16-byte aligned");
    return normalize_dispatch(cfg, h, rows, C, n, nrm, filt, (hipStream_t)stream);
}

extern "C" int sngnn_normalize_rows(const float *h, int64_t rows, int C, float *n, float *nrm, void *stream)
{
    return sngnn_normalize_rows_filter(h, rows, C, n, nrm, nullptr, stream);
}

template <int GF>
static __global__ __launch_bounds__(BLOCK) void k_filter_pair_scores(const uint4 *__restrict__ filt,
                                                                     const int64_t *__restrict__ pa,
                                                                     const int64_t *__restrict__ pb, int64_t n_pairs,
                                                                     float *__restrict__ out)
{
    constexpr int NGF = 64 / GF;
    const int lane = lane_id();
    const int gid = lane / GF, lf = lane % GF;
    const int64_t w = (int64_t)blockIdx.x * WAVES + (threadIdx.x >> 6);
    const int64_t p = w * NGF + gid;
    const int64_t q = p < n_pairs ? p : n_pairs - 1;
    const uint4 fa = filt[(size_t)pa[q] * GF + lf], fb = filt[(size_t)pb[q] * GF + lf];
    const float s = group_sum<GF>(fdot8(fa, fb)) * FILT_UNSCALE;
    if (p < n_pairs && lf == 0) out[p] = s;
}

extern "C" int sngnn_filter_pair_scores(const void *filt, int C, const int64_t *pair_a, const int64_t *pair_b,
                                        int64_t n_pairs, float *out, void *stream)
{
    SN_REQUIRE(filter_row_bytes(C) > 0, SNGNN_EINVAL, "no filter rows for this C");
    SN_REQUIRE(n_pairs >= 0, SNGNN_EINVAL, "negative pair count");
    if (n_pairs == 0) return SNGNN_OK;
    SN_REQUIRE(filt && pair_a && pair_b && out, SNGNN_EINVAL, "NULL argument");
    hipStream_t st = (hipStream_t)stream;
    const int gf = (int)(filter_row_bytes(C) / 16);
    const int grid = ceil_div(n_pairs, (64 / gf) * WAVES);
    const uint4 *f = (const uint4 *)filt;
    switch (gf) {
    case 8: k_filter_pair_scores<8><<<grid, BLOCK, 0, st>>>(f, pair_a, pair_b, n_pairs, out); break;
    case 16: k_filter_pair_scores<16><<<grid, BLOCK, 0, st>>>(f, pair_a, pair_b, n_pairs, out); break;
    case 32: k_filter_pair_scores<32><<<grid, BLOCK, 0, st>>>(f, pair_a, pair_b, n_pairs, out); break;
    default: k_filter_pair_scores<64><<<grid, BLOCK, 0, st>>>(f, pair_a, pair_b, n_pairs, out); break;
    }
    SN_HIP(hipGetLastError());
    return SNGNN_OK;
}

struct FwdCall {
    const sngnn_graph_t *g;
    const void *rows;
    int dtype = 0;
    bool prepared = false;
    const float *nrm = nullptr;
    const void *filt = nullptr;
    bool by_rows = false;
    const uint8_t *row_flag = nullptr;
    int row_want = 0;
    int C, top_k;
    float thr;
    const sngnn_epilogue_t *epi = nullptr;
    void *out;
    float *wsel, *inv_norm;
    int32_t *sel_src = nullptr;
    float *sel_w = nullptr;
    void *workspace, *stream;
};

static int launch_forward(const FwdCall &c, const RowCfg &cfg, const float *n, const float *nrm, const void *filt,
                          hipEvent_t *ev)
{
    const sngnn_graph_t *g = c.g;
    const sngnn_epilogue_t *epi = c.epi;
    const int C = c.C;
    const float thr = c.thr;
    hipStream_t st = (hipStream_t)c.stream;
    const int top_k = std::min(c.top_k, 1 << 20);

    if (c.sel_src && top_k > 0 && c.row_flag == nullptr) {
        const int64_t nw = g->N * (int64_t)top_k;
        k_fill_sel<<<(int)std::min<int64_t>((nw + 255) / 256, 2048), 256, 0, st>>>(c.sel_src, c.sel_w, nw);
    }

    FwdArgs a;
    a.n = n; a.nrm = nrm; a.C = C; a.N = (int)g->N; a.row_off = (int)g->row_off;
    const int64_t table_bytes = g->Ntot * (int64_t)C * (c.dtype == 0 ? 4 : 2);
    const bool buf = c.dtype == 0 && fwd_buffer_form(table_bytes, std::max<int64_t>(4 * g->Ep, 16 * g->N), g_addr_mode);
    a.Ntot = (int)g->Ntot; a.n_bytes = buf ? (unsigned)table_bytes : 0u;
    a.filt = nrm ? (const uint4 *)filt : nullptr;
    a.filt_min_deg = g_filt_min_deg >= 0 ? g_filt_min_deg : (thr >= 0.25f ? 0 : FILT_MIN_DEG);
    a.filt_small = (a.filt != nullptr && top_k >= 0 && g_filter_mode != 0 &&
                    ((thr >= 0.25f && top_k >= 4) || g_filter_mode == 2)) ? 1 : 0;
    a.delta = (float)(4 * C + 32) * 5.9604644775390625e-8f;
    a.role_mask = g_role_mask;
    a.row_flag = c.row_flag; a.row_want = c.row_want;
    a.epi_flags = 0; a.epi_bias = nullptr; a.epi_keep = nullptr; a.epi_seed = nullptr; a.epi_p = 0.f; a.epi_scale = 1.0f;
    a.head_y = nullptr; a.head_sel = nullptr; a.head_part = nullptr; a.head_flags = 0; a.head_nmain = 0;
    a.head_scale = a.head_scale_b = 0.f; a.head_out = nullptr;
    a.kbits = nullptr; a.kb_wbase = (int)g->kb_wbase; a.kb_tbase = (int)g->kb_tbase;
    if (epi && epi->kept_bits) {
        SN_REQUIRE(sngnn::kept_bits_path(g, top_k) && c.row_flag == nullptr && nrm != nullptr, SNGNN_EINVAL,
                   "no kept-bit path for this graph / top_k (sngnn_agg_kept_bits_supported)");
        a.kbits = (unsigned *)epi->kept_bits;
    }
    const bool head = epi != nullptr && epi->head_y != nullptr;
    if (head) {
        SN_REQUIRE(cfg.vec == 4 && cfg.r == 1 && cfg.g <= 16, SNGNN_EINVAL,
                   "the head epilogue needs C % 4 == 0 and C <= 64 (sngnn_agg_head_supported)");
        SN_REQUIRE(epi->head_sel && epi->head_metrics && epi->head_workspace, SNGNN_EINVAL,
                   "head_sel / head_metrics / head_workspace is NULL");
        SN_REQUIRE(epi->head_sets == 1 || epi->head_sets == 2, SNGNN_EINVAL, "head_sets must be 1 or 2");
        SN_REQUIRE((epi->head_out_mode == 1 || epi->head_out_mode == 2) && (epi->head_out_mode != 2 || epi->head_sets == 1),
                   SNGNN_EINVAL, "head_out_mode: 1 logits, 2 gradient (one split only)");
        SN_REQUIRE(c.out != nullptr, SNGNN_EINVAL, "out is NULL");
        SN_REQUIRE(!epi->relu && epi->keep == nullptr && epi->seed == nullptr, SNGNN_EINVAL,
                   "the head follows the LAST layer: no relu / dropout with it");
        SN_REQUIRE(c.row_flag == nullptr && c.sel_src == nullptr, SNGNN_EINVAL,
                   "the head epilogue covers all rows of a call and emits no selection lists");
        a.head_y = epi->head_y; a.head_sel = epi->head_sel;
        a.head_part = (float *)epi->head_workspace; a.head_out = epi->head_metrics;
        a.head_flags = (epi->head_sets == 2 ? 1 : 0) | (epi->head_out_mode == 2 ? 2 : 0);
        a.head_scale = 1.0f / (float)(epi->head_n_a > 0 ? epi->head_n_a : 1);
        a.head_scale_b = 1.0f / (float)(epi->head_n_b > 0 ? epi->head_n_b : 1);
    }
    if (epi) {
        a.epi_bias = epi->bias; a.epi_keep = epi->keep;
        a.epi_seed = (const unsigned long long *)epi->seed; a.epi_p = epi->p;
        const bool drops = epi->keep != nullptr || epi->seed != nullptr;
        a.epi_scale = drops ? epi->keep_scale : 1.0f;
        a.epi_flags = (epi->relu ? 1 : 0) | (epi->bias ? 2 : 0) | (epi->keep ? 4 : (epi->seed ? 8 : 0));
    }
    const bool stream_small = top_k < 0 || top_k >= SMALL_T;
    a.rowptr = g->rowptr; a.col = g->col;
    a.col_s = stream_small ? g->col_s_b : g->col_s;
    a.rperm = stream_small ? g->rperm_b : g->rperm;
    a.rdesc = stream_small ? g->rdesc_b : g->rdesc;
    a.k = top_k < 0 ? -1 : top_k; a.thr = thr;
    a.out = (float *)c.out; a.wsel = c.wsel; a.inv_norm = c.inv_norm;
    a.sel_src = top_k > 0 ? c.sel_src : nullptr; a.sel_w = top_k > 0 ? c.sel_w : nullptr;
    bind_side(g, false, a);
    a.task_order = g->task_order;
    a.split_soff = g->split_soff;
    const FwdLayout L = fwd_layout(g, C);
    char *ws = (char *)c.workspace;
    a.scores = ws ? (float *)(ws + L.scores) : nullptr;
    a.partial = ws ? (float *)(ws + L.partial) : nullptr;
    a.cand_key = ws ? (unsigned long long *)(ws + L.cand_key) : nullptr;
    a.cand_src = ws ? (int32_t *)(ws + L.cand_src) : nullptr;
    a.fin_done = ws ? (unsigned long long *)(ws + L.fin_done) : nullptr;
    a.fin_nonce = 0ull; a.main_blocks = 0; a.n_edges = (long long)g->Ep;
    a.k_magic = top_k >= 2 ? (unsigned)(0xFFFFFFFFu / (unsigned)top_k + 1u) : 0u;
    const int max_split = g->n_split ? g->rdeg[0] : 0;
    a.use_cand = fwd_use_candidates(a.k, C, max_split) ? 1 : 0;
    SN_REQUIRE(a.kbits == nullptr || a.use_cand, SNGNN_EINVAL,
               "no kept-bit path: this graph's biggest row takes the scratch-score finalize");
    a.n_split_gt_wave = top_k > 0 ? g->rows_gt((int64_t)(128 / std::min(top_k, 128)) * CHUNK)
                                  : (top_k < 0 ? g->rows_gt((int64_t)16 * CHUNK) : 0);
    a.lowbits = 1;
    while ((1ll << a.lowbits) < g->max_in_deg && a.lowbits < 31) ++a.lowbits;
    if (head) {
        SN_REQUIRE(g->n_split == 0 || a.use_cand, SNGNN_EINVAL,
                   "no head epilogue: this graph's biggest row takes the scratch-score finalize (sngnn_agg_head_supported)");
        return buf ? launch_agg_fwd_buf_vec<4>(cfg, a, max_split, ev, st)
                   : launch_agg_fwd_vec<float, 4>(cfg, a, max_split, ev, st);
    }
    if (a.epi_flags != 0) {
        SN_REQUIRE(cfg.vec == 4, SNGNN_EINVAL, "the store epilogue needs C % 4 == 0 (16-byte rows)");
        return buf ? launch_agg_fwd_epi_buf_v4(cfg, a, max_split, ev, st)
                   : launch_agg_fwd_epi_v4(cfg, a, max_split, ev, st);
    }
    if (buf)
        return dispatch_vec(cfg, [&](auto vec) { return launch_agg_fwd_buf_vec<decltype(vec)::value>(cfg, a, max_split, ev, st); });
    return SNGNN_LAUNCH_VEC(launch_agg_fwd_vec, cfg, c.dtype, a, max_split, ev, st);
}

static bool use_filter(const sngnn_graph_t *g, int C, int top_k, float thr)
{
    if (g_filter_mode == 0 || top_k < 0 || filter_row_bytes(C) == 0) return false;
    if ((thr >= 0.25f && top_k >= 4) || g_filter_mode == 2) return true;
    if (thr >= 0.25f || g_filter_mode == 3) return g->rows_gt(std::max(top_k, SMALL_T)) != 0;
    if (g->Ep > 0 && (double)g->prunable_edges(top_k, FILT_MIN_DEG) >= FILT_PRUNABLE_SHARE * (double)g->Ep) return true;
    return false;
}

static int run_forward(const FwdCall &c)
{
    const sngnn_graph_t *g = c.g;
    const sngnn_epilogue_t *epi = c.epi;
    SN_REQUIRE(g != nullptr, SNGNN_EINVAL, "graph is NULL");
    SN_REQUIRE(g->N == 0 || (c.rows != nullptr && c.out != nullptr), SNGNN_EINVAL, "h/out is NULL");
    RowCfg cfg;
    if (int rc = check_rows(c.C, c.dtype, {c.rows, c.out}, cfg)) return rc;
    SN_REQUIRE((c.sel_src == nullptr) == (c.sel_w == nullptr), SNGNN_EINVAL, "sel_src and sel_w go together");
    SN_REQUIRE(c.sel_src == nullptr || c.top_k >= 0, SNGNN_EINVAL, "sel_src needs top_k >= 0");
    hipStream_t st = (hipStream_t)c.stream;
    if (g->N == 0) {
        if (epi != nullptr && epi->head_y != nullptr && epi->head_metrics != nullptr)
            return launch_head_reduce(nullptr, 0, 0.f, 0.f, epi->head_sets == 2 ? 2 : 1, 4, epi->head_metrics, st);
        return SNGNN_OK;
    }
    const bool table = !c.prepared && c.dtype == 0 && !(g_table_mode == 2 || (g_table_mode == 0 && c.top_k < 0));
    const bool pays = (table || (c.prepared && !c.by_rows)) && use_filter(g, c.C, c.top_k, c.thr);
    const bool filter = pays && !(epi && epi->no_filter);
    if (c.by_rows) {
        SN_REQUIRE(c.row_flag != nullptr && c.workspace != nullptr, SNGNN_EINVAL, "row_flag/workspace is NULL");
        SN_REQUIRE(c.nrm != nullptr || c.filt == nullptr, SNGNN_EINVAL, "filter rows go with unit rows + norms");
    } else if (c.prepared) {
        SN_REQUIRE(c.nrm != nullptr, SNGNN_EINVAL, "nrm is NULL");
        SN_REQUIRE(c.workspace != nullptr || (g->n_tasks == 0 && (c.filt != nullptr || !pays)), SNGNN_EINVAL,
                   "workspace is NULL");
    } else {
        SN_REQUIRE(c.workspace != nullptr, SNGNN_EINVAL, "workspace is NULL");
    }
    if (c.prepared) {
        SN_REQUIRE(c.filt == nullptr || filter_row_bytes(c.C) > 0, SNGNN_EINVAL,
                   "no filter rows for this C (sngnn_filter_row_bytes(C) == 0)");
        SN_REQUIRE(((uintptr_t)c.filt % 16) == 0, SNGNN_EINVAL, "filt must be 16-byte aligned");
    }
    const FwdLayout L = fwd_layout(g, c.C);
    char *ws = (char *)c.workspace;
    hipEvent_t *ev = (g_prof_on && !c.by_rows) ? g_prof_ev : nullptr;
    if (ev) SN_HIP(hipEventRecord(ev[0], st));
    const float *n = (const float *)c.rows, *nrm = c.nrm;
    const void *filt = c.by_rows ? c.filt : nullptr;
    if (table) {
        float *unit = (float *)(ws + L.unit), *norms = (float *)(ws + L.nrm);
        void *wf = filter ? ws + L.filt : nullptr;
        for (int rep = 0; rep < (ev ? g_prof_reps : 1); ++rep)
            if (int rc = normalize_dispatch(cfg, n, g->Ntot, c.C, unit, norms, wf, st)) return rc;
        n = unit; nrm = norms; filt = wf;
    } else if (filter) {
        filt = c.filt;
        if (!filt) {
            if (int rc = launch_filter_v4(cfg, n, g->Ntot, c.C, ws + L.filt, st)) return rc;
            filt = ws + L.filt;
        }
    }
    return launch_forward(c, cfg, n, nrm, filt, ev ? ev + 1 : nullptr);
}

extern "C" int sngnn_agg_forward(const sngnn_graph_t *g, const float *h, int C, int top_k,
                                 float thr, float *out, float *wsel, float *inv_norm,
                                 int32_t *sel_src, float *sel_w, void *workspace, void *stream)
{
    FwdCall c;
    c.g = g; c.rows = h; c.C = C; c.top_k = top_k; c.thr = thr; c.out = out; c.wsel = wsel; c.inv_norm = inv_norm;
    c.sel_src = sel_src; c.sel_w = sel_w; c.workspace = workspace; c.stream = stream;
    return run_forward(c);
}

extern "C" int sngnn_agg_forward_half(const sngnn_graph_t *g, const void *h, int dtype, int C, int top_k, float thr,
                                      void *out, float *wsel, float *inv_norm, int32_t *sel_src, float *sel_w,
                                      void *workspace, void *stream)
{
    SN_REQUIRE(dtype == SNGNN_DTYPE_F16 || dtype == SNGNN_DTYPE_BF16, SNGNN_EINVAL,
               "dtype must be SNGNN_DTYPE_F16 or SNGNN_DTYPE_BF16");
    FwdCall c;
    c.g = g; c.rows = h; c.dtype = dtype; c.C = C; c.top_k = top_k; c.thr = thr; c.out = out; c.wsel = wsel;
    c.inv_norm = inv_norm; c.sel_src = sel_src; c.sel_w = sel_w; c.workspace = workspace; c.stream = stream;
    return run_forward(c);
}

extern "C" int64_t sngnn_agg_head_workspace_bytes(const sngnn_graph_t *g)
{
    return g ? ((int64_t)HEAD_ROLE_WAVES_MAX + g->n_split) * 16 + 256 : 0;
}

extern "C" int sngnn_agg_head_supported(const sngnn_graph_t *g, int C, int top_k)
{
    RowCfg cfg;
    if (g == nullptr || !row_cfg(C, cfg) || cfg.vec != 4 || cfg.r != 1 || cfg.g > 16) return 0;
    const int max_split = g->n_split ? g->rdeg[0] : 0;
    return (g->n_split == 0 || fwd_use_candidates(top_k < 0 ? -1 : top_k, C, max_split)) ? 1 : 0;
}

static int check_epilogue(const sngnn_epilogue_t *epi)
{
    SN_REQUIRE(epi != nullptr, SNGNN_EINVAL, "epilogue is NULL");
    SN_REQUIRE((epi->keep == nullptr && epi->seed == nullptr) || (epi->keep_scale > 0.f && epi->keep_scale < 1e30f),
               SNGNN_EINVAL, "keep_scale must be a positive finite number (1 / (1 - p))");
    SN_REQUIRE(epi->seed == nullptr || (epi->p >= 0.f && epi->p < 1.f), SNGNN_EINVAL, "p must be in [0, 1)");
    return SNGNN_OK;
}

extern "C" int sngnn_agg_forward_epilogue(const sngnn_graph_t *g, const float *h, int C, int top_k, float thr,
                                          const sngnn_epilogue_t *epi, float *out, float *wsel, float *inv_norm,
                                          void *workspace, void *stream)
{
    if (int rc = check_epilogue(epi)) return rc;
    FwdCall c;
    c.g = g; c.rows = h; c.C = C; c.top_k = top_k; c.thr = thr; c.epi = epi; c.out = out; c.wsel = wsel;
    c.inv_norm = inv_norm; c.workspace = workspace; c.stream = stream;
    return run_forward(c);
}

extern "C" int sngnn_agg_forward_prepared(const sngnn_graph_t *g, const float *n, const float *nrm,
                                          const void *filt, int C, int top_k, float thr, float *out, float *wsel,
                                          float *inv_norm, int32_t *sel_src, float *sel_w, void *workspace,
                                          void *stream)
{
    FwdCall c;
    c.g = g; c.rows = n; c.prepared = true; c.nrm = nrm; c.filt = filt; c.C = C; c.top_k = top_k; c.thr = thr;
    c.out = out; c.wsel = wsel; c.inv_norm = inv_norm; c.sel_src = sel_src; c.sel_w = sel_w;
    c.workspace = workspace; c.stream = stream;
    return run_forward(c);
}

extern "C" int sngnn_agg_forward_prepared_epilogue(const sngnn_graph_t *g, const float *n, const float *nrm,
                                                   const void *filt, int C, int top_k, float thr,
                                                   const sngnn_epilogue_t *epi, float *out, float *wsel,
                                                   float *inv_norm, void *workspace, void *stream)
{
    if (int rc = check_epilogue(epi)) return rc;
    FwdCall c;
    c.g = g; c.rows = n; c.prepared = true; c.nrm = nrm; c.filt = filt; c.C = C; c.top_k = top_k; c.thr = thr;
    c.epi = epi; c.out = out; c.wsel = wsel; c.inv_norm = inv_norm; c.workspace = workspace; c.stream = stream;
    return run_forward(c);
}

extern "C" int sngnn_agg_forward_rows(const sngnn_graph_t *g, const float *n, const float *nrm, const void *filt,
                                      int C, int top_k, float thr, const uint8_t *row_flag, int row_want,
                                      float *out, float *wsel, float *inv_norm, void *workspace, void *stream)
{
    FwdCall c;
    c.g = g; c.rows = n; c.prepared = true; c.nrm = nrm; c.filt = filt; c.by_rows = true; c.row_flag = row_flag;
    c.row_want = row_want; c.C = C; c.top_k = top_k; c.thr = thr; c.out = out; c.wsel = wsel; c.inv_norm = inv_norm;
    c.workspace = workspace; c.stream = stream;
    return run_forward(c);
}

extern "C" int sngnn_agg_kept_bits_supported(const sngnn_graph_t *g, int C, int top_k)
{
    if (!sngnn::kept_bits_path(g, top_k)) return 0;
    return fwd_use_candidates(top_k, C, g->n_split ? g->rdeg[0] : 0) ? 1 : 0;
}

extern "C" int sngnn_filter_wanted(const sngnn_graph_t *g, int C, int top_k, float thr)
{
    return g != nullptr && use_filter(g, C, top_k, thr) ? 1 : 0;
}

extern "C" int sngnn_agg_forward_normalized(const sngnn_graph_t *g, const float *n, const float *nrm, int C,
                                            int top_k, float thr, float *out, float *wsel, float *inv_norm,
                                            int32_t *sel_src, float *sel_w, void *workspace, void *stream)
{
    return sngnn_agg_forward_prepared(g, n, nrm, nullptr, C, top_k, thr, out, wsel, inv_norm, sel_src, sel_w,
                                      workspace, stream);
}
```

### sngnn_amd/csrc/attn.hip

```cpp
#include "attn_impl.h"
#include "entry.h"

using namespace sngnn;

static int forward_impl(const sngnn_graph_t *g, const float *h, int dtype, int C, float *out, float *alpha,
                        void *workspace, void *stream)
{
    SN_REQUIRE(g != nullptr, SNGNN_EINVAL, "graph is NULL");
    if (g->N == 0) return SNGNN_OK;
    SN_REQUIRE(h && out, SNGNN_EINVAL, "NULL argument");
    SN_REQUIRE(workspace != nullptr || g->n_tasks == 0, SNGNN_EINVAL, "workspace is NULL");
    RowCfg cfg;
    if (int rc = check_rows(C, dtype, {h, out}, cfg)) return rc;
    AttnArgs a;
    a.h = h; a.C = C; a.N = (int)g->N; a.row_off = (int)g->row_off;
    a.col = g->col; a.rdesc = g->rdesc;
    a.out = out; a.alpha = alpha;
    bind_side(g, false, a);
    a.partial = workspace ? (float *)((char *)workspace + attn_fwd_layout(g->n_tasks, C).partial) : nullptr;
    a.nbA = a.nbB = 0;
    return SNGNN_LAUNCH_VEC(launch_attn_fwd_vec, cfg, dtype, a, (hipStream_t)stream);
}

extern "C" int sngnn_attn_forward(const sngnn_graph_t *g, const float *h, int C, float *out,
                                  float *alpha, void *workspace, void *stream)
{
    return forward_impl(g, h, 0, C, out, alpha, workspace, stream);
}

extern "C" int sngnn_attn_forward_half(const sngnn_graph_t *g, const void *h, int dtype, int C, void *out,
                                       float *alpha, void *workspace, void *stream)
{
    SN_REQUIRE(dtype == SNGNN_DTYPE_F16 || dtype == SNGNN_DTYPE_BF16, SNGNN_EINVAL,
               "dtype must be SNGNN_DTYPE_F16 or SNGNN_DTYPE_BF16");
    return forward_impl(g, (const float *)h, dtype, C, (float *)out, alpha, workspace, stream);
}

static int backward_impl(const sngnn_graph_t *g, const float *h, int dtype, int C, const float *grad_out,
                         const float *alpha, float *grad_h, void *workspace, void *stream)
{
    SN_REQUIRE(g != nullptr, SNGNN_EINVAL, "graph is NULL");
    if (g->Ntot == 0) return SNGNN_OK;
    SN_REQUIRE(h && grad_h && workspace && (grad_out || g->N == 0), SNGNN_EINVAL, "NULL argument");
    SN_REQUIRE(alpha != nullptr || g->Ep == 0, SNGNN_EINVAL, "alpha is NULL");
    RowCfg cfg;
    if (int rc = check_rows(C, dtype, {h, grad_out, grad_h}, cfg)) return rc;
    const BwdLayout L = bwd_layout(g, C, true);
    BwdArgs a;
    bind_bwd_graph(g, C, L, workspace, a);
    a.h = h; a.gout = grad_out; a.wsel = alpha; a.grad_h = grad_h;
    a.wd = (float2 *)((char *)workspace + L.rec);
    a.rec_dot = (float *)((char *)workspace + L.rec_dot);
    a.kmask = nullptr; a.kmask_words = 0; a.inv_deg = nullptr;
    a.mode = 1; a.top_k = -1; a.role_mask = 3; a.s_small_end = (int)g->Ntot;
    a.fdesc = nullptr; a.trest = nullptr; a.n_fused = a.n_trest = 0;
    a.kbits = nullptr; a.csc_bit = nullptr; a.kb_wbase = a.kb_tbase = 0;
    return SNGNN_LAUNCH_VEC(launch_attn_bwd_vec, cfg, dtype, a, (hipStream_t)stream);
}

extern "C" int sngnn_attn_backward(const sngnn_graph_t *g, const float *h, int C,
                                   const float *grad_out, const float *alpha, float *grad_h,
                                   void *workspace, void *stream)
{
    return backward_impl(g, h, 0, C, grad_out, alpha, grad_h, workspace, stream);
}

extern "C" int sngnn_attn_backward_half(const sngnn_graph_t *g, const void *h, int dtype, int C, const void *grad_out,
                                        const float *alpha, void *grad_h, void *workspace, void *stream)
{
    SN_REQUIRE(dtype == SNGNN_DTYPE_F16 || dtype == SNGNN_DTYPE_BF16, SNGNN_EINVAL,
               "dtype must be SNGNN_DTYPE_F16 or SNGNN_DTYPE_BF16");
    return backward_impl(g, (const float *)h, dtype, C, (const float *)grad_out, alpha, (float *)grad_h, workspace,
                         stream);
}
```

### sngnn_amd/csrc/common.h

```cpp
#pragma once
#include <hip/hip_runtime.h>
#include <stdint.h>
#include <algorithm>
#include <string>
#include <type_traits>
#include <vector>

#include "sngnn_hip.h"
#include "ws_layout.h"

namespace sngnn {

constexpr float EPS_NORM = 1e-12f;

void set_error(const std::string &msg);
int hip_fail(hipError_t e, const char *what, const char *file, int line);

#define SN_HIP(expr)                                                       \
    do {                                                                   \
        hipError_t _e = (expr);                                            \
        if (_e != hipSuccess) return sngnn::hip_fail(_e, #expr, __FILE__, __LINE__); \
    } while (0)

#define SN_REQUIRE(cond, code, msg)                                        \
    do {                                                                   \
        if (!(cond)) { sngnn::set_error(msg); return (code); }             \
    } while (0)

constexpr int WGRAD_MFMA_WGS = 256;
int wgrad_mfma_partials(int64_t N, int C, int F);
int launch_wgrad_mfma(const float *g, const float *x, int64_t N, int C, int F, float *part, float *part_b,
                      hipStream_t st);

int gat_att_blocks(int64_t N);
int launch_gat_scores(const float *xp, int64_t ld, const float *att_src, const float *att_dst, int64_t lda, int64_t N,
                      int H, int C, float *a_src, float *a_dst, hipStream_t st);
int launch_gat_att_part(const float *xp, int64_t ld, const float *gasrc, const float *gadst, int64_t N, int H, int C,
                        double *part, hipStream_t st);
int launch_gat_att_red(const double *part, int64_t N, int H, int C, bool split, float *grad_att, hipStream_t st);

bool kept_bits_path(const sngnn_graph_t *g, int top_k);
bool fwd_scores_on_the_fly_forced();
int set_bwd_mode(int v);
int set_bwd_roles(int v);
int set_lin_mode(int v);
int set_knn_route(int v);
int set_cosine_split(int v);
int set_hist_copies(int v);
bool fp32_mfma_only();

struct RowCfg { int vec, g, r; };
inline bool row_cfg(int C, RowCfg &cfg)
{
    if (C < 1 || C > SNGNN_MAX_CHANNELS) return false;
    int vec = (C % 4 == 0) ? 4 : (C % 2 == 0) ? 2 : 1;
    int lanes = C / vec;
    int g = 8;
    while (g < lanes && g < 64) g <<= 1;
    int r = (lanes + g - 1) / g;
    int rr = 1;
    while (rr < r) rr <<= 1;
    if (rr > 8) return false;
    cfg = {vec, g, rr};
    return true;
}

}

namespace sngnn {
template <typename F> int dispatch_gr(const RowCfg &cfg, F &&f)
{
    using std::integral_constant;
    switch (cfg.g * 100 + cfg.r) {
    case 801: return f(integral_constant<int, 8>{}, integral_constant<int, 1>{});
    case 1601: return f(integral_constant<int, 16>{}, integral_constant<int, 1>{});
    case 3201: return f(integral_constant<int, 32>{}, integral_constant<int, 1>{});
    case 6401: return f(integral_constant<int, 64>{}, integral_constant<int, 1>{});
    case 6402: return f(integral_constant<int, 64>{}, integral_constant<int, 2>{});
    case 6404: return f(integral_constant<int, 64>{}, integral_constant<int, 4>{});
    case 6408: return f(integral_constant<int, 64>{}, integral_constant<int, 8>{});
    default: set_error("unsupported channel layout"); return SNGNN_EINVAL;
    }
}
}
#define SNGNN_DISPATCH_GR(FN, VEC, cfg, ...)                                                                           \
    return sngnn::dispatch_gr(cfg, [&](auto g, auto r) { return FN<VEC, decltype(g)::value, decltype(r)::value>(__VA_ARGS__); });
#define SNGNN_DISPATCH_GRS(FN, VEC, S, cfg, ...)                                                                       \
    return sngnn::dispatch_gr(cfg, [&](auto g, auto r) { return FN<VEC, decltype(g)::value, decltype(r)::value, S>(__VA_ARGS__); });

struct sngnn_graph {
    int64_t N = 0, E_in = 0, Ep = 0;
    int64_t Ntot = 0, row_off = 0;
    int add_loops = 0, remove_loops = 0;
    int32_t *rowptr = nullptr, *col = nullptr, *eid = nullptr;
    int32_t *cscptr = nullptr, *csc_eid = nullptr, *csc_dst = nullptr;
    int32_t *csc_pos = nullptr;
    int32_t *rperm = nullptr, *sperm = nullptr;
    int4 *rdesc = nullptr;
    int32_t *col_s = nullptr;
    int32_t *rperm_b = nullptr, *col_s_b = nullptr;
    int4 *rdesc_b = nullptr;
    int4 *sdesc = nullptr;
    float *inv_deg = nullptr;
    int32_t *csc_bit = nullptr;
    int64_t kb_wbase = 0, kb_tbase = 0, kb_words = 0;
    int4 *fdesc = nullptr;
    int4 *trest = nullptr;
    int n_fused = 0, n_trest = 0;
    int32_t *task_slot = nullptr, *task_chunk = nullptr;
    int32_t *task_order = nullptr;
    int32_t *split_soff = nullptr;
    int32_t *split_task0 = nullptr;
    int32_t *stask_slot = nullptr, *stask_chunk = nullptr;
    int32_t *ssplit_task0 = nullptr;
    std::vector<int32_t> rdeg;
    std::vector<int64_t> rdeg_wave_psum;
    std::vector<int32_t> sdeg;
    int64_t max_in_deg = 0, max_out_deg = 0, src_min = 0;
    int n_split = 0, n_tasks = 0;
    int64_t split_edges = 0;
    int n_ssplit = 0, n_stasks = 0;
    int device = 0;

    int rows_gt(int64_t t) const
    {
        int lo = 0, hi = (int)rdeg.size();
        while (lo < hi) { int m = (lo + hi) / 2; if (rdeg[m] > t) lo = m + 1; else hi = m; }
        return lo;
    }
    int64_t prunable_edges(int top_k, int min_deg) const
    {
        const int64_t t = std::max<int64_t>(std::max<int64_t>(top_k, (int64_t)min_deg - 1), (int64_t)sngnn::SMALL_T);
        const int m = rows_gt(t);
        if (m <= 0 || (size_t)m >= rdeg_wave_psum.size()) return 0;
        return rdeg_wave_psum[(size_t)m] - (int64_t)std::max(top_k, 0) * m;
    }
    int srcs_gt(int64_t t) const
    {
        int lo = 0, hi = (int)sdeg.size();
        while (lo < hi) { int m = (lo + hi) / 2; if (sdeg[m] > t) lo = m + 1; else hi = m; }
        return lo;
    }
};
```

### sngnn_amd/csrc/signed.hip

```cpp
#include "signed_impl.h"
#include "entry.h"

using namespace sngnn;

static int forward_impl(const sngnn_graph_t *g, const float *wh, int dtype, int C, const float *coef, const float *c2,
                        float *out, float *s, void *workspace, void *stream)
{
    SN_REQUIRE(g != nullptr, SNGNN_EINVAL, "graph is NULL");
    if (g->N == 0) return SNGNN_OK;
    SN_REQUIRE(wh && out && c2 && (coef || g->Ep == 0), SNGNN_EINVAL, "NULL argument");
    SN_REQUIRE(workspace != nullptr || g->n_tasks == 0, SNGNN_EINVAL, "workspace is NULL");
    RowCfg cfg;
    if (int rc = check_rows(C, dtype, {wh, out}, cfg)) return rc;
    SignedArgs a;
    a.h = wh; a.coef = coef; a.c2 = c2; a.C = C; a.N = (int)g->N; a.row_off = (int)g->row_off;
    a.col = g->col; a.rdesc = g->rdesc;
    a.out = out; a.s = s;
    bind_side(g, false, a);
    a.partial = workspace ? (float *)((char *)workspace + signed_fwd_layout(g->n_tasks, C).partial) : nullptr;
    a.nbA = a.nbB = 0;
    return SNGNN_LAUNCH_VEC(launch_signed_fwd_vec, cfg, dtype, a, (hipStream_t)stream);
}

extern "C" int sngnn_signed_forward(const sngnn_graph_t *g, const float *wh, int C, const float *coef,
                                    const float *c2, float *out, float *s, void *workspace, void *stream)
{
    return forward_impl(g, wh, 0, C, coef, c2, out, s, workspace, stream);
}

extern "C" int sngnn_signed_forward_half(const sngnn_graph_t *g, const void *wh, int dtype, int C, const float *coef,
                                         const float *c2, void *out, float *s, void *workspace, void *stream)
{
    SN_REQUIRE(dtype == SNGNN_DTYPE_F16 || dtype == SNGNN_DTYPE_BF16, SNGNN_EINVAL,
               "dtype must be SNGNN_DTYPE_F16 or SNGNN_DTYPE_BF16");
    return forward_impl(g, (const float *)wh, dtype, C, coef, c2, (float *)out, s, workspace, stream);
}

static int backward_impl(const sngnn_graph_t *g, const float *wh, int dtype, int C, const float *grad_out,
                         const float *coef, const float *s, const float *c2, float *grad_wh, float *u,
                         void *workspace, void *stream)
{
    SN_REQUIRE(g != nullptr, SNGNN_EINVAL, "graph is NULL");
    if (g->Ntot == 0) return SNGNN_OK;
    SN_REQUIRE(wh && grad_wh && workspace && c2 && (grad_out || g->N == 0), SNGNN_EINVAL, "NULL argument");
    SN_REQUIRE((coef && s && u) || g->Ep == 0, SNGNN_EINVAL, "coef / s / u is NULL");
    RowCfg cfg;
    if (int rc = check_rows(C, dtype, {wh, grad_out, grad_wh}, cfg)) return rc;
    const BwdLayout L = bwd_layout(g, C, true);
    BwdArgs a;
    bind_bwd_graph(g, C, L, workspace, a);
    a.h = wh; a.gout = grad_out; a.wsel = s; a.grad_h = grad_wh;
    a.wd = (float2 *)((char *)workspace + L.rec); a.rec_dot = nullptr;
    a.kmask = nullptr; a.kmask_words = 0; a.inv_deg = nullptr;
    a.mode = 1; a.top_k = -1; a.role_mask = 3; a.s_small_end = (int)g->Ntot;
    a.fdesc = nullptr; a.trest = nullptr; a.n_fused = a.n_trest = 0;
    a.kbits = nullptr; a.csc_bit = nullptr; a.kb_wbase = a.kb_tbase = 0;
    SignedBwdExtra x;
    x.coef = coef; x.c2 = c2; x.u = u;
    return SNGNN_LAUNCH_VEC(launch_signed_bwd_vec, cfg, dtype, a, x, (hipStream_t)stream);
}

extern "C" int sngnn_signed_backward(const sngnn_graph_t *g, const float *wh, int C, const float *grad_out,
                                     const float *coef, const float *s, const float *c2, float *grad_wh, float *u,
                                     void *workspace, void *stream)
{
    return backward_impl(g, wh, 0, C, grad_out, coef, s, c2, grad_wh, u, workspace, stream);
}

extern "C" int sngnn_signed_backward_half(const sngnn_graph_t *g, const void *wh, int dtype, int C,
                                          const void *grad_out, const float *coef, const float *s, const float *c2,
                                          void *grad_wh, float *u, void *workspace, void *stream)
{
    SN_REQUIRE(dtype == SNGNN_DTYPE_F16 || dtype == SNGNN_DTYPE_BF16, SNGNN_EINVAL,
               "dtype must be SNGNN_DTYPE_F16 or SNGNN_DTYPE_BF16");
    return backward_impl(g, (const float *)wh, dtype, C, (const float *)grad_out, coef, s, c2, (float *)grad_wh, u,
                         workspace, stream);
}
```

Baseline: 19.28 billion edges/s.

## Use AMD buffer-resource loads in node-centric backward with dead-lane skipping

```diff
diff --git a/include/sngnn_hip.h b/include/sngnn_hip.h
--- a/include/sngnn_hip.h
+++ b/include/sngnn_hip.h
@@ -94,6 +94,7 @@
                            float *inv_norm, void *workspace, void *stream);
 int sngnn_tuning_set(int which, int value);
 int sngnn_last_forward_finalize_workgroups(void);
+int sngnn_last_backward_buffer_form(void);
 int sngnn_filter_pair_scores(const void *filt, int C, const int64_t *pair_a, const int64_t *pair_b,
                              int64_t n_pairs, float *out, void *stream);
 int sngnn_agg_forward_normalized(const sngnn_graph_t *g, const float *n, const float *nrm,
diff --git a/sngnn_amd/_lib.py b/sngnn_amd/_lib.py
--- a/sngnn_amd/_lib.py
+++ b/sngnn_amd/_lib.py
@@ -40,7 +40,7 @@
     "sngnn_filter_wanted": (_i32, [_vp, _i32, _i32, _f32]),
     "sngnn_agg_forward_rows": (_i32, [_vp, _vp, _vp, _vp, _i32, _i32, _f32, _vp, _i32, _vp, _vp, _vp, _vp, _vp]),
     "sngnn_tuning_set": (_i32, [_i32, _i32]),
-    "sngnn_last_forward_finalize_workgroups": (_i32, []),
+    "sngnn_last_forward_finalize_workgroups": (_i32, []), "sngnn_last_backward_buffer_form": (_i32, []),
     "sngnn_filter_pair_scores": (_i32, [_vp, _i32, _vp, _vp, _i64, _vp, _vp]),
     "sngnn_agg_forward_normalized": (_i32, [_vp, _vp, _vp, _i32, _i32, _f32, _vp, _vp, _vp, _vp, _vp, _vp, _vp]),
     "sngnn_agg_backward": (_i32, [_vp, _vp, _i32, _vp, _vp, _vp, _vp, _vp]),
diff --git a/sngnn_amd/csrc/agg_bwd.hip b/sngnn_amd/csrc/agg_bwd.hip
--- a/sngnn_amd/csrc/agg_bwd.hip
+++ b/sngnn_amd/csrc/agg_bwd.hip
@@ -1,11 +1,16 @@
 #include "agg_bwd_impl.h"
+#include "bwd_plan.h"
 #include "entry.h"
 
 using namespace sngnn;
 
 static int g_bwd_mode = 0, g_bwd_roles = 3;
 int sngnn::set_bwd_mode(int v) { g_bwd_mode = (v == 1 || v == 2) ? v : 0; return SNGNN_OK; }
-int sngnn::set_bwd_roles(int v) { g_bwd_roles = v & 7; return SNGNN_OK; }
+int sngnn::set_bwd_roles(int v) { g_bwd_roles = v & (SNGNN_BWD_EXP ? 7 : 3); return SNGNN_OK; }
+static int g_bwd_addr_mode = 0;
+int sngnn::set_bwd_addr_mode(int v) { g_bwd_addr_mode = v == 1 ? 1 : 0; return SNGNN_OK; }
+static int g_last_bwd_form = -1;
+extern "C" int sngnn_last_backward_buffer_form(void) { return g_last_bwd_form; }
 
 extern "C" int sngnn_agg_backward(const sngnn_graph_t *g, const float *h, int C,
                                   const float *grad_out, const float *wsel, float *grad_h,
@@ -76,6 +81,9 @@
     a.mode = node_centric(g) ? 0 : 1;
     a.top_k = top_k;
     a.role_mask = g_bwd_roles;
+    a.buf = bwd_buffer_form(dtype, (int64_t)g->Ntot * 4 * C, (int64_t)g->N * 4 * C, bwd_index_bytes(g->Ep, g->N),
+                            g_bwd_addr_mode) ? 1 : 0;
+    g_last_bwd_form = a.buf;
     a.fdesc = g->fdesc; a.trest = g->trest;
     a.n_fused = g->n_fused; a.n_trest = g->n_trest;
     a.kbits = kbits; a.csc_bit = g->csc_bit; a.kb_wbase = (int)g->kb_wbase; a.kb_tbase = (int)g->kb_tbase;
diff --git a/sngnn_amd/csrc/agg_bwd_args.h b/sngnn_amd/csrc/agg_bwd_args.h
--- /dev/null
+++ b/sngnn_amd/csrc/agg_bwd_args.h
@@ -0,0 +1,43 @@
+#pragma once
+#include "device_utils.h"
+
+namespace sngnn {
+
+struct BwdArgs {
+    const float *h, *gout, *wsel;
+    int C, N, Ntot, row_off;
+    const int32_t *rowptr, *col, *rperm;
+    const int4 *rdesc, *sdesc;
+    const int32_t *cscptr, *csc_eid, *csc_dst, *csc_pos, *sperm;
+    float2 *wd;
+    float *rec_dot;
+    unsigned *kmask;
+    int64_t kmask_words, Ep;
+    const float *inv_deg;
+    float *dnT, *grad_h;
+    int n_split, n_med_end, n_tasks;
+    const int32_t *task_slot, *task_chunk, *split_task0;
+    float *partT;
+    int n_ssplit, n_smed_end, n_stasks;
+    const int32_t *stask_slot, *stask_chunk, *ssplit_task0;
+    float *partS;
+    int nbA, nbB;
+    int s_small_end;
+    const int4 *fdesc;
+    const int4 *trest;
+    int n_fused, n_trest, nbC;
+    int mode;
+    int buf;
+    int role_mask;
+    int top_k;
+    const unsigned *kbits;
+    const int32_t *csc_bit;
+    int kb_wbase, kb_tbase;
+    template <typename S> __device__ __forceinline__ const S *hrows() const { return reinterpret_cast<const S *>(h); }
+    template <typename S> __device__ __forceinline__ const S *grows() const { return reinterpret_cast<const S *>(gout); }
+    template <typename S> __device__ __forceinline__ S *dhrows() const { return reinterpret_cast<S *>(grad_h); }
+};
+
+__device__ __forceinline__ bool kbit(const BwdArgs &a, int b) { return (a.kbits[b >> 5] >> (b & 31)) & 1u; }
+
+}
diff --git a/sngnn_amd/csrc/agg_bwd_flat_v1.hip b/sngnn_amd/csrc/agg_bwd_flat_v1.hip
--- /dev/null
+++ b/sngnn_amd/csrc/agg_bwd_flat_v1.hip
@@ -0,0 +1,3 @@
+#include "agg_bwd_impl.h"
+
+SNGNN_AGG_BWD_NODE_TU(false, 1)
diff --git a/sngnn_amd/csrc/agg_bwd_flat_v2.hip b/sngnn_amd/csrc/agg_bwd_flat_v2.hip
--- /dev/null
+++ b/sngnn_amd/csrc/agg_bwd_flat_v2.hip
@@ -0,0 +1,3 @@
+#include "agg_bwd_impl.h"
+
+SNGNN_AGG_BWD_NODE_TU(false, 2)
diff --git a/sngnn_amd/csrc/agg_bwd_flat_v4.hip b/sngnn_amd/csrc/agg_bwd_flat_v4.hip
--- /dev/null
+++ b/sngnn_amd/csrc/agg_bwd_flat_v4.hip
@@ -0,0 +1,3 @@
+#include "agg_bwd_impl.h"
+
+SNGNN_AGG_BWD_NODE_TU(false, 4)
diff --git a/sngnn_amd/csrc/agg_bwd_impl.h b/sngnn_amd/csrc/agg_bwd_impl.h
--- a/sngnn_amd/csrc/agg_bwd_impl.h
+++ b/sngnn_amd/csrc/agg_bwd_impl.h
@@ -1,47 +1,14 @@
 #pragma once
-#include "device_utils.h"
+#include "agg_bwd_src.h"
 
 #ifndef SNGNN_BWDF_STEP
 #define SNGNN_BWDF_STEP 1
 #endif
+#ifndef SNGNN_BWD_EXP
+#define SNGNN_BWD_EXP 0
+#endif
 
 namespace sngnn {
-
-struct BwdArgs {
-    const float *h, *gout, *wsel;
-    int C, N, Ntot, row_off;
-    const int32_t *rowptr, *col, *rperm;
-    const int4 *rdesc, *sdesc;
-    const int32_t *cscptr, *csc_eid, *csc_dst, *csc_pos, *sperm;
-    float2 *wd;
-    float *rec_dot;
-    unsigned *kmask;
-    int64_t kmask_words, Ep;
-    const float *inv_deg;
-    float *dnT, *grad_h;
-    int n_split, n_med_end, n_tasks;
-    const int32_t *task_slot, *task_chunk, *split_task0;
-    float *partT;
-    int n_ssplit, n_smed_end, n_stasks;
-    const int32_t *stask_slot, *stask_chunk, *ssplit_task0;
-    float *partS;
-    int nbA, nbB;
-    int s_small_end;
-    const int4 *fdesc;
-    const int4 *trest;
-    int n_fused, n_trest, nbC;
-    int mode;
-    int role_mask;
-    int top_k;
-    const unsigned *kbits;
-    const int32_t *csc_bit;
-    int kb_wbase, kb_tbase;
-    template <typename S> __device__ __forceinline__ const S *hrows() const { return reinterpret_cast<const S *>(h); }
-    template <typename S> __device__ __forceinline__ const S *grows() const { return reinterpret_cast<const S *>(gout); }
-    template <typename S> __device__ __forceinline__ S *dhrows() const { return reinterpret_cast<S *>(grad_h); }
-};
-
-__device__ __forceinline__ bool kbit(const BwdArgs &a, int b) { return (a.kbits[b >> 5] >> (b & 31)) & 1u; }
 
 __device__ __forceinline__ bool is_kept(float w) { return w > -3.0f; }
 
@@ -296,6 +263,15 @@
     const float dse = group_sum<G>(gi.dot_partial(hv)) * invdeg;
     fma_row<VEC, G, R>(msg, w * invdeg * live, gi);
     fma_row<VEC, G, R>(dns, dse * invi * live, x);
+}
+
+__device__ __forceinline__ int bwd_exp_one(const BwdArgs &a, int i)
+{
+#if SNGNN_BWD_EXP
+    return (a.role_mask & 4) ? 0 : i;
+#else
+    return i;
+#endif
 }
 
 template <int VEC, int G, int R>
@@ -373,7 +349,7 @@
             s_edge_rows<VEC, G, R>(x0, g0, w0, ds0, msg, dns);
             s_edge_rows<VEC, G, R>(x1, g1, two ? w1 : 0.f, two ? ds1 : 0.f, msg, dns);
         } else {
-            const float d0 = a.inv_deg[(a.role_mask & 4) ? 0 : i0], d1 = a.inv_deg[(a.role_mask & 4) ? 0 : i1];
+            const float d0 = a.inv_deg[bwd_exp_one(a, i0)], d1 = a.inv_deg[bwd_exp_one(a, i1)];
             s_edge_recompute<VEC, G, R>(x0, g0, fin.hv, invv, d0, 1.0f, msg, dns);
             s_edge_recompute<VEC, G, R>(x1, g1, fin.hv, invv, d1, two ? 1.0f : 0.0f, msg, dns);
         }
@@ -381,40 +357,38 @@
     s_finish<VEC, G, R, S>(a, v, lg, msg, dns, fin);
 }
 
-template <int VEC, int G, int R, bool KB = false, typename S = float>
-__device__ __forceinline__ void f_role_node(const BwdArgs &a, int blk, int *lds_wave)
+template <int VEC, int G, int R, bool KB = false, typename S = float, typename Src>
+__device__ __forceinline__ void f_role_node(const BwdArgs &a, const Src &src, int blk, int *lds_wave)
 {
     using RowT = Row<VEC, G, R>;
     constexpr int RPW = 64 / G;
     const int lane = lane_id(), wave = threadIdx.x >> 6;
     const int gid = lane / G, lg = lane % G;
     const int slot = (blk * WAVES + wave) * RPW + gid;
-    if (slot >= a.n_fused) return;
-    const int4 d = a.fdesc[slot];
+    const bool have = slot < a.n_fused;
+    if (!Src::skips_dead && !have) return;
+    const int4 d = src.fdesc(slot);
     const int v = d.x, rs = d.y, qs = d.z, deg = d.w & 255, od = d.w >> 8;
     const int vl = v - a.row_off;
     int *s_j = lds_wave + gid * 2 * SMALL_T;
     int *s_i = s_j + SMALL_T;
     FinishRows<VEC, G, R, S> fin;
     RowT gp;
-    gp.load(a.grows<S>() + (size_t)vl * a.C, a.C, lg);
-    fin.hv.load(a.hrows<S>() + (size_t)v * a.C, a.C, lg);
+    src.grow_if(gp, vl, have);
+    src.hrow_if(fin.hv, v, have);
     fin.own = true;
     int nk = 0, nko = 0;
     unsigned hw = 0u;
-    if constexpr (KB) hw = reinterpret_cast<const unsigned short *>(a.kbits)[vl];
+    if constexpr (KB) hw = reinterpret_cast<const unsigned short *>(a.kbits)[have ? vl : 0];
     for (int t0 = 0; t0 < max(deg, od); t0 += G) {
         const int t = t0 + lg;
         bool kept_i;
         if constexpr (KB) kept_i = t < deg && ((hw >> t) & 1u);
         else kept_i = t < deg && kept_csr(a, rs + t);
-        const int j = t < deg ? a.col[rs + t] : 0;
+        const int j = src.col_if(rs + t, t < deg);
         bool kept_o = false;
-        int it = 0;
-        if (t < od) {
-            it = a.csc_dst[qs + t];
-            kept_o = kept_out<KB>(a, qs + t);
-        }
+        const int it = src.dst_if(qs + t, t < od);
+        if (t < od) kept_o = kept_out<KB>(a, qs + t);
         const unsigned long long gi = group_bits<G>(__ballot(kept_i), gid);
         const unsigned long long go = group_bits<G>(__ballot(kept_o), gid);
         const unsigned long long below = (1ull << lg) - 1ull;
@@ -431,8 +405,8 @@
     dns.zero();
     wave_lds_sync();
     constexpr int FU = SNGNN_BWDF_STEP;
-    const int steps = (max(nk, nko) + FU - 1) / FU;
-    for (int s = 0; s < steps; ++s) {
+    auto step = [&](int s, auto in_c, auto out_c) {
+        constexpr bool IN = decltype(in_c)::value, OUT = decltype(out_c)::value;
         RowT xj[FU], x[FU], gi[FU];
         float dd[FU];
         bool ti[FU], to[FU];
@@ -441,20 +415,39 @@
             const int q = FU * s + u;
             ti[u] = q < nk;
             to[u] = q < nko;
-            const int j = ti[u] ? s_j[q] : v;
-            const int i = to[u] ? s_i[q] : vl;
-            xj[u].load(a.hrows<S>() + (size_t)j * a.C, a.C, lg);
-            x[u].load(a.hrows<S>() + (size_t)(i + a.row_off) * a.C, a.C, lg);
-            gi[u].load(a.grows<S>() + (size_t)i * a.C, a.C, lg);
-            dd[u] = a.inv_deg[i];
-        }
-#pragma unroll
-        for (int u = 0; u < FU; ++u) t_edge_row<VEC, G, R>(xj[u], gp, fin.t, ti[u] ? 1.0f : 0.0f);
-#pragma unroll
-        for (int u = 0; u < FU; ++u)
-            s_edge_recompute<VEC, G, R>(x[u], gi[u], fin.hv, invv, dd[u], to[u] ? 1.0f : 0.0f, msg, dns);
-    }
-    s_finish<VEC, G, R, S>(a, v, lg, msg, dns, fin);
+            if constexpr (IN) src.hrow_if(xj[u], src.pick(ti[u], s_j[q], v), ti[u]);
+            if constexpr (OUT) {
+                const int i = src.pick(to[u], s_i[q], vl);
+                src.hrow_if(x[u], i + a.row_off, to[u]);
+                src.grow_if(gi[u], i, to[u]);
+                dd[u] = src.inv_deg_if(i, to[u]);
+            }
+        }
+        if constexpr (IN)
+#pragma unroll
+            for (int u = 0; u < FU; ++u) t_edge_row<VEC, G, R>(xj[u], gp, fin.t, src.live_w(ti[u]));
+        if constexpr (OUT)
+#pragma unroll
+            for (int u = 0; u < FU; ++u)
+                s_edge_recompute<VEC, G, R>(x[u], gi[u], fin.hv, invv, dd[u], src.live_w(to[u]), msg, dns);
+    };
+    if constexpr (Src::skips_dead) {
+        int wk = 0, wko = 0;
+#pragma unroll
+        for (int gq = 0; gq < RPW; ++gq) {
+            wk = max(wk, __builtin_amdgcn_readlane(nk, gq * G));
+            wko = max(wko, __builtin_amdgcn_readlane(nko, gq * G));
+        }
+        const int si = (wk + FU - 1) / FU, so = (wko + FU - 1) / FU;
+        int s = 0;
+        for (; s < min(si, so); ++s) step(s, std::true_type{}, std::true_type{});
+        for (; s < si; ++s) step(s, std::true_type{}, std::false_type{});
+        for (; s < so; ++s) step(s, std::false_type{}, std::true_type{});
+    } else {
+        const int steps = (max(nk, nko) + FU - 1) / FU;
+        for (int s = 0; s < steps; ++s) step(s, std::true_type{}, std::true_type{});
+    }
+    if (have) s_finish<VEC, G, R, S>(a, v, lg, msg, dns, fin);
 }
 
 __device__ __forceinline__ int wave_prefix_incl(int v)
@@ -468,8 +461,8 @@
     return v;
 }
 
-template <int VEC, int G, int R, bool KB = false, typename S = float>
-__device__ __forceinline__ void w_role_node(const BwdArgs &a, int blk, int *lds_wave)
+template <int VEC, int G, int R, bool KB = false, typename S = float, typename Src>
+__device__ __forceinline__ void w_role_node(const BwdArgs &a, const Src &src, int blk, int *lds_wave)
 {
     using RowT = Row<VEC, G, R>;
     constexpr int NG = 64 / G;
@@ -477,14 +470,14 @@
     const int gid = lane / G, lg = lane % G;
     const int slot = blk * WAVES + wave;
     if (slot >= a.n_med_end + a.n_trest) return;
-    const int4 d = slot < a.n_med_end ? a.rdesc[slot] : a.trest[slot - a.n_med_end];
+    const int4 d = src.wdesc(slot);
     const int vl = d.x, rs = d.y, deg = d.z;
     const int v = vl + a.row_off;
     const int qs = a.cscptr[v], od = a.cscptr[v + 1] - qs;
     FinishRows<VEC, G, R, S> fin;
     RowT gp;
-    gp.load(a.grows<S>() + (size_t)vl * a.C, a.C, lg);
-    fin.hv.load(a.hrows<S>() + (size_t)v * a.C, a.C, lg);
+    src.grow(gp, vl);
+    src.hrow(fin.hv, v);
     fin.own = true;
     gp.scale(1.0f / (float)max(deg, 1));
     fin.t.zero();
@@ -495,16 +488,22 @@
     auto flush = [&]() {
         wave_lds_sync();
         if (!have_ids) {
-            for (int t = lane; t < n; t += 64) elist[t] = a.col[(KB ? rs : 0) + elist[t]];
+            for (int t = lane; t < n; t += 64) elist[t] = src.col_if((KB ? rs : 0) + elist[t], true);
             wave_lds_sync();
         }
         for (int q0 = 0; q0 < n; q0 += 2 * NG) {
             const int qa = min(q0 + gid, n - 1), qb = min(q0 + NG + gid, n - 1);
+            const bool la = q0 + gid < n, lb = q0 + NG + gid < n;
             RowT xa, xb;
-            xa.load(a.hrows<S>() + (size_t)elist[qa] * a.C, a.C, lg);
-            xb.load(a.hrows<S>() + (size_t)elist[qb] * a.C, a.C, lg);
-            t_edge_row<VEC, G, R>(xa, gp, fin.t, q0 + gid < n ? 1.0f : 0.0f);
-            t_edge_row<VEC, G, R>(xb, gp, fin.t, q0 + NG + gid < n ? 1.0f : 0.0f);
+            if (!Src::skips_dead || q0 + NG < n) {
+                src.hrow_if(xa, elist[qa], la);
+                src.hrow_if(xb, elist[qb], lb);
+                t_edge_row<VEC, G, R>(xa, gp, fin.t, src.live_w(la));
+                t_edge_row<VEC, G, R>(xb, gp, fin.t, src.live_w(lb));
+            } else {
+                src.hrow_if(xa, elist[qa], la);
+                t_edge_row<VEC, G, R>(xa, gp, fin.t, src.live_w(la));
+            }
         }
         wave_lds_sync();
         n = 0;
@@ -528,7 +527,7 @@
             bool kept;
             if constexpr (KB) kept = t < deg && kbit(a, bitbase + t);
             else kept = t < deg && kept_csr(a, rs + t);
-            const int j = t < deg ? a.col[rs + t] : 0;
+            const int j = src.col_if(rs + t, t < deg);
             const unsigned long long m = __ballot(kept);
             if (kept) elist[n + prefix_popc(m)] = j;
             n += __popcll(m);
@@ -568,7 +567,7 @@
     if (s_here)
         for (int base = 0; base < od; base += 64) {
             const int t = base + lane;
-            const int it = t < od ? a.csc_dst[qs + t] : 0;
+            const int it = src.dst_if(qs + t, t < od);
             const bool kept = t < od && kept_out<KB>(a, qs + t);
             const unsigned long long m = __ballot(kept);
             if (kept) s_i[nso + prefix_popc(m)] = it;
@@ -590,13 +589,20 @@
         const bool la = q0 + gid < nso, lb = q0 + NG + gid < nso;
         const int ia = s_i[qa], ib = s_i[qb];
         RowT xa, ga, xb, gb;
-        xa.load(a.hrows<S>() + (size_t)(ia + a.row_off) * a.C, a.C, lg);
-        ga.load(a.grows<S>() + (size_t)ia * a.C, a.C, lg);
-        xb.load(a.hrows<S>() + (size_t)(ib + a.row_off) * a.C, a.C, lg);
-        gb.load(a.grows<S>() + (size_t)ib * a.C, a.C, lg);
-        const float da = a.inv_deg[ia], db = a.inv_deg[ib];
-        s_edge_recompute<VEC, G, R>(xa, ga, fin.hv, invv, da, la ? 1.0f : 0.0f, msg, dns);
-        s_edge_recompute<VEC, G, R>(xb, gb, fin.hv, invv, db, lb ? 1.0f : 0.0f, msg, dns);
+        if (!Src::skips_dead || q0 + NG < nso) {
+            src.hrow_if(xa, ia + a.row_off, la);
+            src.grow_if(ga, ia, la);
+            src.hrow_if(xb, ib + a.row_off, lb);
+            src.grow_if(gb, ib, lb);
+            const float da = src.inv_deg_if(ia, la), db = src.inv_deg_if(ib, lb);
+            s_edge_recompute<VEC, G, R>(xa, ga, fin.hv, invv, da, src.live_w(la), msg, dns);
+            s_edge_recompute<VEC, G, R>(xb, gb, fin.hv, invv, db, src.live_w(lb), msg, dns);
+        } else {
+            src.hrow_if(xa, ia + a.row_off, la);
+            src.grow_if(ga, ia, la);
+            const float da = src.inv_deg_if(ia, la);
+            s_edge_recompute<VEC, G, R>(xa, ga, fin.hv, invv, da, src.live_w(la), msg, dns);
+        }
     }
     msg.reduce_across_groups();
     dns.reduce_across_groups();
@@ -622,28 +628,30 @@
 }
 
 #define SNGNN_BWDF_ATTR __attribute__((amdgpu_waves_per_eu(R == 1 ? 8 : 1, 8)))
-template <int VEC, int G, int R, bool KB = false, typename S = float>
+template <int VEC, int G, int R, bool KB = false, typename S = float, bool BUF = false>
 __global__ __launch_bounds__(BLOCK) SNGNN_BWDF_ATTR void k_bwd_w(const BwdArgs a)
 {
     __shared__ __align__(16) int lds[WAVES][2 * WAVE_T];
     const int b = blockIdx.x;
     int *lw = lds[threadIdx.x >> 6];
+    const BwdSrc<BUF, VEC, G, R, S> src(a, lane_id() % G);
     const int stride = a.nbB;
     const int cw = min(a.nbA, (b + stride - 1) / stride);
-    if (b % stride == 0 && b / stride < a.nbA) { if (a.role_mask & 1) w_role_node<VEC, G, R, KB, S>(a, b / stride, lw); }
-    else if (a.role_mask & 2) f_role_node<VEC, G, R, KB, S>(a, b - cw, lw);
-}
-
-template <int VEC, int G, int R, typename S = float>
+    if (b % stride == 0 && b / stride < a.nbA) { if (a.role_mask & 1) w_role_node<VEC, G, R, KB, S>(a, src, b / stride, lw); }
+    else if (a.role_mask & 2) f_role_node<VEC, G, R, KB, S>(a, src, b - cw, lw);
+}
+
+template <int VEC, int G, int R, typename S = float, bool BUF = false>
 __global__ __launch_bounds__(BLOCK) SNGNN_BWDF_ATTR void k_bwd_f(const BwdArgs a)
 {
     __shared__ __align__(16) int lds[WAVES][256];
     const int b = blockIdx.x;
     int *lw = lds[threadIdx.x >> 6];
+    const BwdSrc<BUF, VEC, G, R, S> src(a, lane_id() % G);
     if (b < a.nbA) t_role_wave<VEC, G, R, false, S>(a, b, lw, true);
     else if (b < a.nbA + a.nbB) t_role_wave<VEC, G, R, false, S>(a, b - a.nbA, lw, false);
     else if (b < a.nbA + a.nbB + a.nbC) t_role_small<VEC, G, R, false, S>(a, b - a.nbA - a.nbB, lw, a.trest, a.n_trest);
-    else f_role_node<VEC, G, R, false, S>(a, b - a.nbA - a.nbB - a.nbC, lw);
+    else f_role_node<VEC, G, R, false, S>(a, src, b - a.nbA - a.nbB - a.nbC, lw);
 }
 
 template <int VEC, int G, int R, bool REC, bool CSRM, typename S = float>
@@ -725,7 +733,7 @@
             s_edge_rows<VEC, G, R>(xa, ga, ra.x, ra.y, msg, dns);
             s_edge_rows<VEC, G, R>(xb, gb, rb.x, rb.y, msg, dns);
         } else {
-            const float da = a.inv_deg[(a.role_mask & 4) ? 0 : ia], db = a.inv_deg[(a.role_mask & 4) ? 0 : ib];
+            const float da = a.inv_deg[bwd_exp_one(a, ia)], db = a.inv_deg[bwd_exp_one(a, ib)];
             s_edge_recompute<VEC, G, R>(xa, ga, hv, invv, da, la ? 1.0f : 0.0f, msg, dns);
             s_edge_recompute<VEC, G, R>(xb, gb, hv, invv, db, lb ? 1.0f : 0.0f, msg, dns);
         }
@@ -784,6 +792,29 @@
     for (int64_t i = blockIdx.x * (int64_t)blockDim.x + threadIdx.x; i < n; i += (int64_t)gridDim.x * blockDim.x) p[i] = 0u;
 }
 
+template <bool BUF, int VEC> int launch_bwd_node_vec(const RowCfg &cfg, const BwdArgs &a, int which, int grid, hipStream_t st);
+
+template <int VEC, int G, int R, bool BUF> int launch_bwd_node(const BwdArgs &a, int which, int grid, hipStream_t st)
+{
+    if (which == 1) k_bwd_f<VEC, G, R, float, BUF><<<grid, BLOCK, 0, st>>>(a);
+    else if (a.kbits) k_bwd_w<VEC, G, R, true, float, BUF><<<grid, BLOCK, 0, st>>>(a);
+    else k_bwd_w<VEC, G, R, false, float, BUF><<<grid, BLOCK, 0, st>>>(a);
+    return SNGNN_OK;
+}
+
+template <int VEC, int G, int R, typename S> void launch_bwd_node_any(const BwdArgs &a, int which, int grid, hipStream_t st)
+{
+    if constexpr (std::is_same<S, float>::value) {
+        const RowCfg cfg{VEC, G, R};
+        if (a.buf) launch_bwd_node_vec<true, VEC>(cfg, a, which, grid, st);
+        else launch_bwd_node_vec<false, VEC>(cfg, a, which, grid, st);
+    } else {
+        if (which == 1) k_bwd_f<VEC, G, R, S><<<grid, BLOCK, 0, st>>>(a);
+        else if (a.kbits) k_bwd_w<VEC, G, R, true, S><<<grid, BLOCK, 0, st>>>(a);
+        else k_bwd_w<VEC, G, R, false, S><<<grid, BLOCK, 0, st>>>(a);
+    }
+}
+
 template <int VEC, int G, int R, typename S = float> int launch_agg_bwd(const BwdArgs &a0, hipStream_t st)
 {
     constexpr int RPW = 64 / G;
@@ -799,10 +830,7 @@
             a.nbA = ceil_div(a.n_med_end + a.n_trest, WAVES);
             const int nbF = ceil_div(a.n_fused, (int64_t)WAVES * RPW);
             a.nbB = std::max(1, (a.nbA + nbF) / std::max(a.nbA, 1));
-            if (a.nbA + nbF > 0) {
-                if (a.kbits) k_bwd_w<VEC, G, R, true, S><<<a.nbA + nbF, BLOCK, 0, st>>>(a);
-                else k_bwd_w<VEC, G, R, false, S><<<a.nbA + nbF, BLOCK, 0, st>>>(a);
-            }
+            if (a.nbA + nbF > 0) launch_bwd_node_any<VEC, G, R, S>(a, 0, a.nbA + nbF, st);
             if (a.n_stasks > 0) {
                 a.nbA = ceil_div(a.n_stasks, WAVES);
                 a.nbB = 0;
@@ -816,7 +844,7 @@
         a.nbB = ceil_div(a.n_med_end - a.n_split, WAVES);
         a.nbC = ceil_div(a.n_trest, (int64_t)WAVES * RPW);
         const int nbD = ceil_div(a.n_fused, (int64_t)WAVES * RPW);
-        if (a.nbA + a.nbB + a.nbC + nbD > 0) k_bwd_f<VEC, G, R, S><<<a.nbA + a.nbB + a.nbC + nbD, BLOCK, 0, st>>>(a);
+        if (a.nbA + a.nbB + a.nbC + nbD > 0) launch_bwd_node_any<VEC, G, R, S>(a, 1, a.nbA + a.nbB + a.nbC + nbD, st);
         if (a.n_split > 0) k_bwd_t_fin<<<a.n_split, 256, 0, st>>>(a);
         a.nbA = ceil_div(a.n_stasks, WAVES);
         a.nbB = ceil_div(a.n_smed_end - a.n_ssplit, WAVES);
@@ -846,6 +874,15 @@
 
 }
 
+#define SNGNN_AGG_BWD_NODE_TU(BUF, VEC)                                                                                \
+    template <>                                                                                                        \
+    int sngnn::launch_bwd_node_vec<BUF, VEC>(const RowCfg &cfg, const BwdArgs &a, int which, int grid, hipStream_t st) \
+    {                                                                                                                  \
+        return sngnn::dispatch_gr(cfg, [&](auto g, auto r) {                                                           \
+            return launch_bwd_node<VEC, decltype(g)::value, decltype(r)::value, BUF>(a, which, grid, st);              \
+        });                                                                                                            \
+    }
+
 #define SNGNN_AGG_BWD_TU(S, VEC)                                                                                       \
     template <> int sngnn::launch_agg_bwd_vec<S, VEC>(const RowCfg &cfg, const BwdArgs &a, hipStream_t st)             \
     {                                                                                                                  \
diff --git a/sngnn_amd/csrc/agg_bwd_src.h b/sngnn_amd/csrc/agg_bwd_src.h
--- /dev/null
+++ b/sngnn_amd/csrc/agg_bwd_src.h
@@ -0,0 +1,99 @@
+#pragma once
+#include "agg_bwd_args.h"
+
+namespace sngnn {
+
+template <bool BUF, int VEC, int G, int R, typename S> struct BwdSrc;
+
+template <int VEC, int G, int R, typename S> struct BwdSrc<false, VEC, G, R, S> {
+    using RowT = Row<VEC, G, R>;
+    static constexpr bool skips_dead = false;
+    const BwdArgs &a;
+    int lg;
+    __device__ __forceinline__ BwdSrc(const BwdArgs &a_, int lg_) : a(a_), lg(lg_) {}
+    __device__ __forceinline__ int pick(bool live, int j, int self) const { return live ? j : self; }
+    __device__ __forceinline__ float live_w(bool live) const { return live ? 1.0f : 0.0f; }
+    __device__ __forceinline__ void hrow(RowT &x, int j) const { x.load(a.template hrows<S>() + (size_t)j * a.C, a.C, lg); }
+    __device__ __forceinline__ void hrow_if(RowT &x, int j, bool) const { hrow(x, j); }
+    __device__ __forceinline__ void grow(RowT &x, int i) const { x.load(a.template grows<S>() + (size_t)i * a.C, a.C, lg); }
+    __device__ __forceinline__ void grow_if(RowT &x, int i, bool) const { grow(x, i); }
+    __device__ __forceinline__ float inv_deg_if(int i, bool) const { return a.inv_deg[i]; }
+    __device__ __forceinline__ int col_if(int e, bool live) const { return live ? a.col[e] : 0; }
+    __device__ __forceinline__ int dst_if(int q, bool live) const { return live ? a.csc_dst[q] : 0; }
+    __device__ __forceinline__ int4 fdesc(int slot) const { return a.fdesc[slot]; }
+    __device__ __forceinline__ int4 wdesc(int slot) const
+    {
+        return slot < a.n_med_end ? a.rdesc[slot] : a.trest[slot - a.n_med_end];
+    }
+};
+
+template <int VEC, int G, int R> struct BwdSrc<true, VEC, G, R, float> {
+    using RowT = Row<VEC, G, R>;
+    static constexpr bool skips_dead = true;
+    __amdgpu_buffer_rsrc_t r_h, r_g, r_col, r_dst, r_invdeg, r_fdesc, r_rdesc, r_trest;
+    unsigned row_bytes;
+    int n_med_end;
+    unsigned loff[R];
+    __device__ __forceinline__ BwdSrc(const BwdArgs &a, int lg)
+    {
+        row_bytes = (unsigned)a.C * 4u;
+        r_h = make_rsrc(a.h, (unsigned)a.Ntot * row_bytes);
+        r_g = make_rsrc(a.gout, (unsigned)a.N * row_bytes);
+        r_col = make_rsrc(a.col, (unsigned)a.Ep * 4u);
+        r_dst = make_rsrc(a.csc_dst, (unsigned)a.Ep * 4u);
+        r_invdeg = make_rsrc(a.inv_deg, (unsigned)a.N * 4u);
+        r_fdesc = make_rsrc(a.fdesc, (unsigned)a.n_fused * 16u);
+        r_rdesc = make_rsrc(a.rdesc, (unsigned)a.N * 16u);
+        r_trest = make_rsrc(a.trest, (unsigned)a.n_trest * 16u);
+        n_med_end = a.n_med_end;
+#pragma unroll
+        for (int r = 0; r < R; ++r) {
+            const int c0 = (r * G + lg) * VEC;
+            loff[r] = c0 < a.C ? (unsigned)c0 * 4u : BUF_OOB;
+        }
+    }
+    __device__ __forceinline__ int pick(bool, int j, int) const { return j; }
+    __device__ __forceinline__ float live_w(bool) const { return 1.0f; }
+    __device__ __forceinline__ void row_at(RowT &x, __amdgpu_buffer_rsrc_t t, unsigned ro) const
+    {
+        unsigned off[R];
+#pragma unroll
+        for (int r = 0; r < R; ++r) off[r] = ro + loff[r];
+        x.load_buf(t, off);
+    }
+    __device__ __forceinline__ void row_at_if(RowT &x, __amdgpu_buffer_rsrc_t t, unsigned ro, bool live) const
+    {
+        unsigned off[R];
+#pragma unroll
+        for (int r = 0; r < R; ++r) off[r] = buf_off_add_sat(live ? ro : BUF_OOB, loff[r]);
+        x.load_buf(t, off);
+    }
+    __device__ __forceinline__ void hrow(RowT &x, int j) const { row_at(x, r_h, (unsigned)j * row_bytes); }
+    __device__ __forceinline__ void hrow_if(RowT &x, int j, bool live) const { row_at_if(x, r_h, (unsigned)j * row_bytes, live); }
+    __device__ __forceinline__ void grow(RowT &x, int i) const { row_at(x, r_g, (unsigned)i * row_bytes); }
+    __device__ __forceinline__ void grow_if(RowT &x, int i, bool live) const { row_at_if(x, r_g, (unsigned)i * row_bytes, live); }
+    __device__ __forceinline__ float inv_deg_if(int i, bool live) const
+    {
+        return __uint_as_float(__builtin_amdgcn_raw_buffer_load_b32(r_invdeg, live ? (unsigned)i * 4u : BUF_OOB, 0, 0));
+    }
+    __device__ __forceinline__ int col_if(int e, bool live) const
+    {
+        return (int)__builtin_amdgcn_raw_buffer_load_b32(r_col, live ? (unsigned)e * 4u : BUF_OOB, 0, 0);
+    }
+    __device__ __forceinline__ int dst_if(int q, bool live) const
+    {
+        return (int)__builtin_amdgcn_raw_buffer_load_b32(r_dst, live ? (unsigned)q * 4u : BUF_OOB, 0, 0);
+    }
+    static __device__ __forceinline__ int4 desc_at(__amdgpu_buffer_rsrc_t t, int slot)
+    {
+        const auto d = __builtin_amdgcn_raw_buffer_load_b128(t, (unsigned)slot * 16u, 0, 0);
+        return make_int4((int)d[0], (int)d[1], (int)d[2], (int)d[3]);
+    }
+    __device__ __forceinline__ int4 fdesc(int slot) const { return desc_at(r_fdesc, slot); }
+    __device__ __forceinline__ int4 wdesc(int slot) const
+    {
+        return slot < n_med_end ? desc_at(r_rdesc, slot) : desc_at(r_trest, slot - n_med_end);
+    }
+};
+
+}
diff --git a/sngnn_amd/csrc/agg_bwd_v1.hip b/sngnn_amd/csrc/agg_bwd_v1.hip
--- a/sngnn_amd/csrc/agg_bwd_v1.hip
+++ b/sngnn_amd/csrc/agg_bwd_v1.hip
@@ -1,3 +1,4 @@
 #include "agg_bwd_impl.h"
 
+SNGNN_AGG_BWD_NODE_TU(true, 1)
 SNGNN_AGG_BWD_TU(float, 1)
diff --git a/sngnn_amd/csrc/agg_bwd_v2.hip b/sngnn_amd/csrc/agg_bwd_v2.hip
--- a/sngnn_amd/csrc/agg_bwd_v2.hip
+++ b/sngnn_amd/csrc/agg_bwd_v2.hip
@@ -1,3 +1,4 @@
 #include "agg_bwd_impl.h"
 
+SNGNN_AGG_BWD_NODE_TU(true, 2)
 SNGNN_AGG_BWD_TU(float, 2)
diff --git a/sngnn_amd/csrc/agg_bwd_v4.hip b/sngnn_amd/csrc/agg_bwd_v4.hip
--- a/sngnn_amd/csrc/agg_bwd_v4.hip
+++ b/sngnn_amd/csrc/agg_bwd_v4.hip
@@ -1,3 +1,4 @@
 #include "agg_bwd_impl.h"
 
+SNGNN_AGG_BWD_NODE_TU(true, 4)
 SNGNN_AGG_BWD_TU(float, 4)
diff --git a/sngnn_amd/csrc/agg_fwd.hip b/sngnn_amd/csrc/agg_fwd.hip
--- a/sngnn_amd/csrc/agg_fwd.hip
+++ b/sngnn_amd/csrc/agg_fwd.hip
@@ -69,7 +69,8 @@
 bool sngnn::fwd_scores_on_the_fly_forced() { return g_table_mode == 2; }
 extern "C" int sngnn_tuning_set(int which, int value)
 {
-    SN_REQUIRE(which == 0 || (which >= 2 && which <= 11), SNGNN_EINVAL, "unknown tuning knob");
+    SN_REQUIRE(which == 0 || (which >= 2 && which <= 12), SNGNN_EINVAL, "unknown tuning knob");
+    if (which == 12) return sngnn::set_bwd_addr_mode(value);
     if (which == 11) { g_addr_mode = value == 1 ? 1 : 0; return SNGNN_OK; }
     if (which == 10) return sngnn::set_hist_copies(value);
     if (which == 9) { sngnn::g_fin_inline = value < 0 ? 0 : value; return SNGNN_OK; }
diff --git a/sngnn_amd/csrc/attn.hip b/sngnn_amd/csrc/attn.hip
--- a/sngnn_amd/csrc/attn.hip
+++ b/sngnn_amd/csrc/attn.hip
@@ -52,7 +52,7 @@
     a.wd = (float2 *)((char *)workspace + L.rec);
     a.rec_dot = (float *)((char *)workspace + L.rec_dot);
     a.kmask = nullptr; a.kmask_words = 0; a.inv_deg = nullptr;
-    a.mode = 1; a.top_k = -1; a.role_mask = 3; a.s_small_end = (int)g->Ntot;
+    a.mode = 1; a.top_k = -1; a.role_mask = 3; a.buf = 0; a.s_small_end = (int)g->Ntot;
     a.fdesc = nullptr; a.trest = nullptr; a.n_fused = a.n_trest = 0;
     a.kbits = nullptr; a.csc_bit = nullptr; a.kb_wbase = a.kb_tbase = 0;
     return SNGNN_LAUNCH_VEC(launch_attn_bwd_vec, cfg, dtype, a, (hipStream_t)stream);
diff --git a/sngnn_amd/csrc/bwd_plan.h b/sngnn_amd/csrc/bwd_plan.h
--- /dev/null
+++ b/sngnn_amd/csrc/bwd_plan.h
@@ -0,0 +1,14 @@
+#pragma once
+#include <stdint.h>
+
+namespace sngnn {
+
+constexpr int64_t BWD_BUFFER_LIMIT = (int64_t)1 << 31;
+inline bool bwd_buffer_form(int dtype, int64_t h_bytes, int64_t g_bytes, int64_t index_bytes, int addr_mode)
+{
+    return dtype == 0 && addr_mode != 1 && h_bytes < BWD_BUFFER_LIMIT && g_bytes < BWD_BUFFER_LIMIT &&
+           index_bytes < BWD_BUFFER_LIMIT;
+}
+inline int64_t bwd_index_bytes(int64_t Ep, int64_t N) { return 4 * Ep > 16 * N ? 4 * Ep : 16 * N; }
+
+}
diff --git a/sngnn_amd/csrc/common.h b/sngnn_amd/csrc/common.h
--- a/sngnn_amd/csrc/common.h
+++ b/sngnn_amd/csrc/common.h
@@ -43,6 +43,7 @@
 bool fwd_scores_on_the_fly_forced();
 int set_bwd_mode(int v);
 int set_bwd_roles(int v);
+int set_bwd_addr_mode(int v);
 int set_lin_mode(int v);
 int set_knn_route(int v);
 int set_cosine_split(int v);
diff --git a/sngnn_amd/csrc/signed.hip b/sngnn_amd/csrc/signed.hip
--- a/sngnn_amd/csrc/signed.hip
+++ b/sngnn_amd/csrc/signed.hip
@@ -52,7 +52,7 @@
     a.h = wh; a.gout = grad_out; a.wsel = s; a.grad_h = grad_wh;
     a.wd = (float2 *)((char *)workspace + L.rec); a.rec_dot = nullptr;
     a.kmask = nullptr; a.kmask_words = 0; a.inv_deg = nullptr;
-    a.mode = 1; a.top_k = -1; a.role_mask = 3; a.s_small_end = (int)g->Ntot;
+    a.mode = 1; a.top_k = -1; a.role_mask = 3; a.buf = 0; a.s_small_end = (int)g->Ntot;
     a.fdesc = nullptr; a.trest = nullptr; a.n_fused = a.n_trest = 0;
     a.kbits = nullptr; a.csc_bit = nullptr; a.kb_wbase = a.kb_tbase = 0;
     SignedBwdExtra x;
```

After: 19.19 billion edges/s. No clear change (-0.5%).
